# LeapLabTHU/LAUDNet

Hardware: AMD Instinct MI355X
Metric: images/sec, LAUD-ResNet101 @224 bs256 (dynamic-inference hot path) (higher is better)
Workload: dtype bf16x3 (fp32 tensors; each fp32 product = 3 bf16 MFMA products of hi/lo splits, fp32 accumulate)

## Files before the change

### include/ldn_hip.h

```cpp
#ifndef LDN_HIP_H
#define LDN_HIP_H

#include <stddef.h>
#include <stdint.h>

#ifdef __cplusplus
extern "C" {
#endif

#define LDN_OK 0
#define LDN_EINVAL (-1)
#define LDN_EHIP (-2)

const char* ldn_last_error(void);
int ldn_version(void);
int ldn_debug_violations(int* count, int* first_code, int reset);
int ldn_plan_timeouts(int* count, int reset);
const int* ldn_fault_flag(void);
int ldn_device_cus(int* cus);
#define LDN_MATH_DEFAULT (-1)
#define LDN_MATH_FP32 0
#define LDN_MATH_BF16X3 1
int ldn_default_math_mode(void);

int ldn_spatial_masker(const float* x, int B, int Hi, int Wi, int C, const float* w ,
                       const float* bias , int g, int S, float* mask, float* logits, float* work,
                       const int32_t* carry_prefix, const float* carry_mask, void* stream);
size_t ldn_spatial_masker_workspace_bytes(int B, int Hi, int Wi, int C, int S);

int ldn_mask_to_index(const float* patch_mask, int B, int Sy, int Sx, int Ho, int Wo, int stride, int32_t* idx3,
                      int32_t* pos3, int32_t* idx1, int32_t* pos1, int32_t* nbr, int32_t* cnt,
                      int32_t* img_prefix3, int32_t* img_prefix1, float* stats, int32_t* work, void* stream);
size_t ldn_mask_to_index_workspace_bytes(int B, int Ho, int Wo, int stride);
int ldn_plan_work_zeroed(int yes);
int ldn_coarsen_cell_means(const float* fine, int B, int S, int C, float* coarse, void* stream);

int ldn_layer_index(const float* image_mask, int B, int Ho, int Wo, int stride, int tile_gy, int tile_gx, int32_t* idx3,
                    int32_t* pos3, int32_t* idx1, int32_t* pos1, int32_t* nbr, int32_t* cnt, int32_t* img_prefix3,
                    int32_t* img_prefix1, float* stats, void* stream);
int ldn_layer_head(const float* pool, int B, int nparts, int C, const float* w , const float* bias , int g,
                   float* mask , float* logits , void* stream);
int ldn_mask_plan_fits(int S, int Sx, int Ho, int Wo, int stride);
int ldn_mask_plan(const float* patch_mask, const float* pool, int C, const float* w, const float* bias, float* mask_out,
                  float* logits, int B, int S, int Sx, int Ho, int Wo, int stride, int patch_major, int32_t* idx3,
                  int32_t* pos3, int32_t* idx1, int32_t* pos1, int32_t* nbr, int32_t* cnt, int32_t* img_prefix3,
                  int32_t* img_prefix1, float* stats, int32_t* work, void* stream);

int ldn_gather_rows(const float* src, int ld_src, const int32_t* rows, const int32_t* count, int cap, int C,
                    float* packed, int ld_packed, void* stream);
int ldn_scatter_add_relu(const float* packed, int ld_packed, const int32_t* rows, const int32_t* count, int cap,
                         int C, const float* identity, int ld_id, float* out, int ld_out, void* stream);

int ldn_conv_rows(const float* a, int lda, const int32_t* a_rows, int taps, const int32_t* m_count, int m_cap,
                  const float* w, int cin, int cout, const float* scale, const float* shift, int relu,
                  const int32_t* relu_if_neg, const int32_t* out_rows, const float* residual, int ldr,
                  float* out, int ldo, int math_mode, void* stream);

int ldn_conv_rows_split(const float* a, int lda, const int32_t* a_rows, int taps, const int32_t* m_count, int m_cap,
                        const void* w_split, int cin, int cout, const float* scale, const float* shift, int relu,
                        const int32_t* relu_if_neg, const int32_t* out_rows, const float* residual, int ldr, float* out,
                        int ldo, const float* post_sub, const float* chan_mask, int rows_per_image, int shift_classes,
                        const int32_t* pix_map, int Hi, int Wi, int Ho, int Wo, int stride, const float* ln_stats,
                        const float* ln_c1, void* stream);
int ldn_conv_rows_f32(const float* a, int lda, const int32_t* a_rows, int taps, const int32_t* m_count, int m_cap,
                        const float* w, int cin, int cout, const float* scale, const float* shift, int relu,
                        const int32_t* relu_if_neg, const int32_t* out_rows, const float* residual, int ldr, float* out,
                        int ldo, const float* post_sub, const float* chan_mask, int rows_per_image, int shift_classes,
                        const int32_t* pix_map, int Hi, int Wi, int Ho, int Wo, int stride, const float* ln_stats,
                        const float* ln_c1, void* stream);

int ldn_hint_rows(int rows);

int ldn_wgrad_rows_ok(int cin, int cout, int taps);
size_t ldn_wgrad_rows_workspace_bytes(int m_cap, int cin, int cout, int taps);
int ldn_wgrad_rows(const float* dy, int lddy, const float* a, int lda, int a_valid, const int32_t* a_rows, int taps,
                   const int32_t* m_count, int m_cap, int cin, int cout, float* dw, float* work, int math_mode, void* stream);

int ldn_rows_chanmask(float* u, int ldu, const int32_t* row_prefix, int B, const float* chan_mask, const int32_t* m_count, int m_cap,
                      int C, void* stream);

size_t ldn_rows_act_bwd_workspace_bytes(int m_cap, int C, int B);
int ldn_rows_act_bwd(const float* dh, int lddh, const float* u, int ldu, const float* post_sub, const float* scale, const float* shift,
                     const float* chan_mask, const int32_t* row_prefix, int B, const float* zy, int ldzy, const int32_t* m_count,
                     int m_cap, int C, float* du, int lddu, float* g_shift, float* g_scale_num, float* g_mask, float* work,
                     void* stream);

int ldn_conv_rows_pool(const float* a, int lda, const int32_t* a_rows, const int32_t* m_count, int m_cap, const void* w,
                       int cin, int cout, const float* scale, const float* shift, int relu, const int32_t* relu_if_neg,
                       const int32_t* out_rows, const float* residual, int ldr, float* out, int ldo, float* pool, int S,
                       int Sx, int Ho, int Wo, int math_mode, void* stream);

int ldn_conv_rows_ps(const float* a, int lda, int a_presplit, const int32_t* a_rows, const int32_t* m_count, int m_cap,
                     const void* w_split, int cin, int cout, const float* scale, const float* shift, int relu,
                     const int32_t* relu_if_neg, const int32_t* out_rows, const float* residual, int ldr, float* out, int ldo,
                     int out_presplit, float* pool, int S, int Sx, int Ho, int Wo, void* stream);
int ldn_conv3x3_rows_ps(const void* a_presplit, int lda, const int32_t* nbr, const int32_t* m_count, int m_cap, const void* w_split,
                        int cin, int cout, const float* scale, const float* shift, int relu, void* out, int ldo, int out_presplit,
                        int rows_hint, void* stream);
int ldn_row_stats(const float* x, int ld, int rows, int C, float eps, float* stats, void* stream);
int ldn_row_stats_list(const float* x, int ld, int rows, int C, float eps, const int32_t* list, const int32_t* count, float* stats,
                       void* stream);

int ldn_channel_masker_splits(int HW);
int ldn_channel_masker(const float* x, int B, int HW, int C, const float* w1, const float* b1, const float* w2,
                       const float* b2, int hidden, int G, int gran, const float* mask_in, float* mask,
                       float* logits, int32_t* ch_idx, int32_t* ch_cnt, float* work, const float* gap_partial,
                       int gap_splits, void* stream);
size_t ldn_channel_masker_workspace_bytes(int B, int HW, int C);

int ldn_forward_stats(const int32_t* cnt, int B, const float* denom, const float* st_in, int st_cols, const double* terms,
                      double static_flops, int n_blocks, float* st_out, float* perc, float* flops, void* stream);

int ldn_conv_image(const float* a, int lda, int B, int Hi, int Wi, int ksize, int stride, int Ho, int Wo,
                   const float* w, int cin, int cout, const int32_t* k_idx, const int32_t* k_cnt, int kgran,
                   const int32_t* n_idx, const int32_t* n_cnt, const float* scale, const float* shift,
                   int shift_classes, const float* post_sub, int relu, const float* residual, int ldr,
                   float* out, int ldo, float* colsum, int out_format, int math_mode, void* stream);

int ldn_bottleneck_head(const float* x, int ldx, int B, int HW, int cin, const void* w1_split, int width,
                        const int32_t* ch_idx, const int32_t* ch_cnt, const float* scale1, const float* shift1,
                        const float* post_sub1, void* h1_split, int ldh, void* stream);
int ldn_bottleneck_head_f32(const float* x, int ldx, int B, int HW, int cin, const float* w1, int width,
                            const int32_t* ch_idx, const int32_t* ch_cnt, const float* scale1, const float* shift1,
                            const float* post_sub1, float* h1, int ldh, void* stream);
int ldn_bottleneck_tail_f32(const void* h1, int ldh, int B, int H, int Wd, int stride, int width, const void* w2_pairs_f32,
                            const void* w3_pairs_f32, int cout, const int32_t* ch_idx, const int32_t* ch_cnt, const float* scale2,
                            const float* shift2_tab, const float* post_sub2, const float* shift3, const float* residual,
                            int ldr, float* out, int ldo, float* colsum, void* stream);
int ldn_bottleneck_tail_splits(int H, int Wd, int width, int stride);
int ldn_bottleneck_tail(const void* h1_split, int ldh, int B, int H, int Wd, int stride, int width, const void* w2_pairs,
                        const void* w3_pairs, int cout, const int32_t* ch_idx, const int32_t* ch_cnt, const float* scale2,
                        const float* shift2_tab, const float* post_sub2, const float* shift3, const float* residual,
                        int ldr, float* out, int ldo, float* colsum, void* stream);
size_t ldn_x_split_bytes(size_t pixels, int cin);
int ldn_bottleneck_head_split(const float* x, int ldx, int B, int HW, int cin, const void* w1_split, int width,
                              const int32_t* ch_idx, const int32_t* ch_cnt, const float* scale1, const float* shift1,
                              const float* post_sub1, void* h1_split, int ldh, void* x_split, void* stream);
int ldn_bottleneck_tail_proj_fits(int H, int Wd, int width, int cin);
int ldn_bottleneck_tail_proj(const void* h1_split, int ldh, int B, int H, int Wd, int width, const void* w2_pairs,
                             const void* w3_pairs, int cout, const int32_t* ch_idx, const int32_t* ch_cnt, const float* scale2,
                             const float* shift2_tab, const float* post_sub2, const float* shift3d, const void* x_split,
                             int cin, const void* wd_pairs, float* out, int ldo, float* colsum, void* stream);

int ldn_bottleneck_smallmap_fits(int H, int Wd, int cin, int width, int cout);
int ldn_bottleneck_smallmap(const float* x, int ldx, int B, int H, int Wd, int cin, int width, const void* w1_split,
                            const void* w2_pairs, const void* w3_pairs, int cout, const int32_t* ch_idx, const int32_t* ch_cnt,
                            const float* scale1, const float* shift1, const float* post_sub1, const float* scale2,
                            const float* shift2_tab, const float* post_sub2, const float* shift3, const float* residual, int ldr,
                            float* out, int ldo, float* colsum, void* stream);

typedef struct ldn_chain_block {
    const void* w1_split; const float* scale1; const float* shift1; const float* post_sub1;
    const void* w2_pairs; const void* w3_pairs; const float* scale2; const float* shift2_tab; const float* post_sub2;
    const float* shift3;
    const float* mw1; const float* mb1; const float* mw2; const float* mb2;
} ldn_chain_block;
int ldn_bottleneck_chain_fits(int H, int Wd, int C, int width, int hidden, int G);
int ldn_bottleneck_chain(const float* x_in, float* x_work, int ldx, int B, int H, int Wd, int C, int width,
                         const ldn_chain_block* blocks, int nblocks, int hidden, int G, int gran, const float* gap_in,
                         int gap_splits, float* colsum, float* masks, int32_t* ch_idx, int32_t* ch_cnt, void* h1_split,
                         int ldh, void* stream);
int ldn_bottleneck_chain_f32(const float* x_in, float* x_work, int ldx, int B, int H, int Wd, int C, int width,
                         const ldn_chain_block* blocks, int nblocks, int hidden, int G, int gran, const float* gap_in,
                         int gap_splits, float* colsum, float* masks, int32_t* ch_idx, int32_t* ch_cnt, float* h1,
                         int ldh, void* stream);

size_t ldn_stem_weight_bytes(int cout);
int ldn_stem_conv_pool(const float* x, int B, int H, int W, const void* w_frag, const float* shift, int cout, float* out,
                       int Hp, int Wp, void* stream);
int ldn_stem_gap_splits(int H, int W);
int ldn_stem_conv_pool_gap(const float* x, int B, int H, int W, const void* w_frag, const float* shift, int cout,
                           float* out, int Hp, int Wp, float* gap, void* stream);

size_t ldn_stem3_weight_bytes(int cout);
int ldn_stem3_conv(const float* x, int B, int H, int W, const void* w_frag, const float* shift, int cout, int relu, float* out,
                   int Ho, int Wo, void* stream);

int ldn_conv_packed(const float* a, int lda, int B, const int32_t* row_prefix, const int32_t* m_count, int m_cap,
                    const int32_t* a_map, int taps, const int32_t* out_map, const int32_t* pix_map, int Hi, int Wi,
                    int Ho, int Wo, int stride, const float* w, int cin, int cout, const int32_t* k_idx,
                    const int32_t* k_cnt, int kgran, const int32_t* n_idx, const int32_t* n_cnt, const float* scale,
                    const float* shift, int shift_classes, const float* post_sub, int relu,
                    const int32_t* relu_if_neg, const float* residual, int ldr, float* out, int ldo, int math_mode,
                    void* stream);

int ldn_grouped_conv3x3_rows(const float* a, int lda, const int32_t* nbr, const int32_t* m_count, int m_cap,
                             const float* w, int C, int group_width, const float* scale, const float* shift, int relu,
                             float* out, int ldo, void* stream);
size_t ldn_grouped16_weight_bytes(int C);
int ldn_grouped16_conv3x3_rows(const float* a, int lda, const int32_t* nbr, const int32_t* m_count, int m_cap,
                               const void* w_frag, int C, const float* scale, const float* shift, int relu, float* out,
                               int ldo, void* stream);

int ldn_grouped16_images_fit(int Hi, int Wi, int C);
int ldn_grouped16_conv3x3_images(const float* a, int lda, const int32_t* m_count, int images_cap, int Hi, int Wi, int Ho, int Wo,
                                 int stride, const void* w_frag, int C, const float* scale, const float* shift, int relu, float* out,
                                 int ldo, void* stream);
int ldn_grouped_conv3x3_image(const float* a, int lda, int B, int Hi, int Wi, int stride, int Ho, int Wo, const float* w,
                              int C, int group_width, const int32_t* ch_idx, const int32_t* ch_cnt, const float* scale,
                              const float* shift, int relu, float* out, int ldo, void* stream);
int ldn_se_packed(float* a, int lda, const int32_t* row_prefix, int B, int C, int S, const float* w1, const float* b1,
                  const float* w2, const float* b2, const int32_t* ch_idx, const int32_t* ch_cnt, int max_rows_per_image,
                  float* work, void* stream);
size_t ldn_se_packed_workspace_bytes(int B, int C, int max_rows_per_image);

int ldn_grouped16_images_bands(int Hi, int Wi, int Ho, int stride, int C);
int ldn_grouped16_conv3x3_images_gap(const float* a, int lda, const int32_t* m_count, int images_cap, int Hi, int Wi, int Ho, int Wo,
                                     int stride, const void* w_frag, int C, const float* scale, const float* shift, int relu, float* out,
                                     int ldo, float* gap_partial, void* stream);
int ldn_se_gate_slots(const float* gap_partial, int splits, const int32_t* m_count, int images_cap, int rows_per_image, int C, int S,
                      const float* w1, const float* b1, const float* w2, const float* b2, float* gate, void* stream);
int ldn_conv_rows_gated(const float* a, int lda, const int32_t* m_count, int m_cap, const void* w_split, int cin, int cout,
                        const float* scale, const float* shift, int relu, const int32_t* relu_if_neg, const int32_t* out_rows,
                        const float* residual, int ldr, float* out, int ldo, const float* gate, int gate_rows, void* stream);

int ldn_packed_mha(const float* qkv, int ld_qkv, const int32_t* tok_rows, const int32_t* img_prefix, int B, int heads,
                   int head_dim, int max_tokens, float scale, float* out, int ldo, void* stream);
int ldn_packed_mha_heads(const float* qkv, int ld_qkv, const int32_t* tok_rows, const int32_t* img_prefix, int B, int heads,
                         int head_dim, int max_tokens, float scale, const float* head_keep, float* out, int ldo, void* stream);

#ifdef __cplusplus
}
#endif
#endif
```

### laudnet_amd/_lib.py

```python
from __future__ import annotations

import ctypes as C
import os

import torch

_PKG = os.path.dirname(os.path.abspath(__file__))
LIB_PATH = os.environ.get("LDN_LIB_PATH", os.path.join(_PKG, "libldn_hip.so"))

_P = C.c_void_p
_I = C.c_int

SIGNATURES = {
    "ldn_last_error": ([], C.c_char_p),
    "ldn_version": ([], _I),
    "ldn_debug_violations": ([C.POINTER(_I), C.POINTER(_I), _I], _I),
    "ldn_plan_timeouts": ([C.POINTER(_I), _I], _I),
    "ldn_fault_flag": ([], C.POINTER(_I)),
    "ldn_device_cus": ([C.POINTER(_I)], _I),
    "ldn_default_math_mode": ([], _I),
    "ldn_spatial_masker": ([_P, _I, _I, _I, _I, _P, _P, _I, _I, _P, _P, _P, _P, _P, _P], _I),
    "ldn_spatial_masker_workspace_bytes": ([_I, _I, _I, _I, _I], C.c_size_t),
    "ldn_mask_to_index": ([_P, _I, _I, _I, _I, _I, _I, _P, _P, _P, _P, _P, _P, _P, _P, _P, _P, _P], _I),
    "ldn_mask_to_index_workspace_bytes": ([_I, _I, _I, _I], C.c_size_t),
    "ldn_mask_plan_fits": ([_I, _I, _I, _I, _I], _I),
    "ldn_hint_rows": ([_I], _I),
    "ldn_layer_index": ([_P, _I, _I, _I, _I, _I, _I, _P, _P, _P, _P, _P, _P, _P, _P, _P, _P], _I),
    "ldn_layer_head": ([_P, _I, _I, _I, _P, _P, _I, _P, _P, _P], _I),
    "ldn_mask_plan": ([_P, _P, _I, _P, _P, _P, _P, _I, _I, _I, _I, _I, _I, _I, _P, _P, _P, _P, _P, _P, _P, _P, _P, _P, _P], _I),
    "ldn_conv_rows_pool": ([_P, _I, _P, _P, _I, _P, _I, _I, _P, _P, _I, _P, _P, _P, _I, _P, _I, _P, _I, _I, _I, _I, _I, _P], _I),
    "ldn_conv_rows_ps": ([_P, _I, _I, _P, _P, _I, _P, _I, _I, _P, _P, _I, _P, _P, _P, _I, _P, _I, _I, _P, _I, _I, _I, _I, _P], _I),
    "ldn_conv3x3_rows_ps": ([_P, _I, _P, _P, _I, _P, _I, _I, _P, _P, _I, _P, _I, _I, _I, _P], _I),
    "ldn_gather_rows": ([_P, _I, _P, _P, _I, _I, _P, _I, _P], _I),
    "ldn_scatter_add_relu": ([_P, _I, _P, _P, _I, _I, _P, _I, _P, _I, _P], _I),
    "ldn_conv_rows": ([_P, _I, _P, _I, _P, _I, _P, _I, _I, _P, _P, _I, _P, _P, _P, _I, _P, _I, _I, _P], _I),
    "ldn_conv_rows_split": ([_P, _I, _P, _I, _P, _I, _P, _I, _I, _P, _P, _I, _P, _P, _P, _I, _P, _I, _P, _P, _I, _I, _P, _I, _I, _I,
                             _I, _I, _P, _P, _P], _I),
    "ldn_conv_rows_f32": ([_P, _I, _P, _I, _P, _I, _P, _I, _I, _P, _P, _I, _P, _P, _P, _I, _P, _I, _P, _P, _I, _I, _P, _I, _I, _I,
                             _I, _I, _P, _P, _P], _I),
    "ldn_wgrad_rows_ok": ([_I, _I, _I], _I),
    "ldn_wgrad_rows_workspace_bytes": ([_I, _I, _I, _I], C.c_size_t),
    "ldn_wgrad_rows": ([_P, _I, _P, _I, _I, _P, _I, _P, _I, _I, _I, _P, _P, _I, _P], _I),
    "ldn_rows_chanmask": ([_P, _I, _P, _I, _P, _P, _I, _I, _P], _I),
    "ldn_rows_act_bwd_workspace_bytes": ([_I, _I, _I], C.c_size_t),
    "ldn_rows_act_bwd": ([_P, _I, _P, _I, _P, _P, _P, _P, _P, _I, _P, _I, _P, _I, _I, _P, _I, _P, _P, _P, _P, _P], _I),
    "ldn_row_stats": ([_P, _I, _I, _I, C.c_float, _P, _P], _I),
    "ldn_row_stats_list": ([_P, _I, _I, _I, C.c_float, _P, _P, _P, _P], _I),
    "ldn_channel_masker_splits": ([_I], _I),
    "ldn_channel_masker": ([_P, _I, _I, _I, _P, _P, _P, _P, _I, _I, _I, _P, _P, _P, _P, _P, _P, _P, _I, _P], _I),
    "ldn_channel_masker_workspace_bytes": ([_I, _I, _I], C.c_size_t),
    "ldn_forward_stats": ([_P, _I, _P, _P, _I, _P, C.c_double, _I, _P, _P, _P, _P], _I),
    "ldn_conv_packed": ([_P, _I, _I, _P, _P, _I, _P, _I, _P, _P, _I, _I, _I, _I, _I, _P, _I, _I, _P, _P, _I, _P, _P, _P, _P,
                         _I, _P, _I, _P, _P, _I, _P, _I, _I, _P], _I),
    "ldn_grouped_conv3x3_rows": ([_P, _I, _P, _P, _I, _P, _I, _I, _P, _P, _I, _P, _I, _P], _I),
    "ldn_grouped16_weight_bytes": ([_I], C.c_size_t),
    "ldn_grouped16_conv3x3_rows": ([_P, _I, _P, _P, _I, _P, _I, _P, _P, _I, _P, _I, _P], _I),
    "ldn_grouped16_images_fit": ([_I, _I, _I], _I),
    "ldn_grouped16_conv3x3_images": ([_P, _I, _P, _I, _I, _I, _I, _I, _I, _P, _I, _P, _P, _I, _P, _I, _P], _I),
    "ldn_plan_work_zeroed": ([_I], _I),
    "ldn_coarsen_cell_means": ([_P, _I, _I, _I, _P, _P], _I),
    "ldn_grouped16_images_bands": ([_I, _I, _I, _I, _I], _I),
    "ldn_grouped16_conv3x3_images_gap": ([_P, _I, _P, _I, _I, _I, _I, _I, _I, _P, _I, _P, _P, _I, _P, _I, _P, _P], _I),
    "ldn_se_gate_slots": ([_P, _I, _P, _I, _I, _I, _I, _P, _P, _P, _P, _P, _P], _I),
    "ldn_conv_rows_gated": ([_P, _I, _P, _I, _P, _I, _I, _P, _P, _I, _P, _P, _P, _I, _P, _I, _P, _I, _P], _I),
    "ldn_grouped_conv3x3_image": ([_P, _I, _I, _I, _I, _I, _I, _I, _P, _I, _I, _P, _P, _P, _P, _I, _P, _I, _P], _I),
    "ldn_se_packed": ([_P, _I, _P, _I, _I, _I, _P, _P, _P, _P, _P, _P, _I, _P, _P], _I),
    "ldn_se_packed_workspace_bytes": ([_I, _I, _I], C.c_size_t),
    "ldn_conv_image": ([_P, _I, _I, _I, _I, _I, _I, _I, _I, _P, _I, _I, _P, _P, _I, _P, _P, _P, _P, _I, _P, _I,
                        _P, _I, _P, _I, _P, _I, _I, _P], _I),
    "ldn_bottleneck_head": ([_P, _I, _I, _I, _I, _P, _I, _P, _P, _P, _P, _P, _P, _I, _P], _I),
    "ldn_bottleneck_head_f32": ([_P, _I, _I, _I, _I, _P, _I, _P, _P, _P, _P, _P, _P, _I, _P], _I),
    "ldn_bottleneck_tail_splits": ([_I, _I, _I, _I], _I),
    "ldn_bottleneck_tail": ([_P, _I, _I, _I, _I, _I, _I, _P, _P, _I, _P, _P, _P, _P, _P, _P, _P, _I, _P, _I, _P, _P], _I),
    "ldn_bottleneck_tail_f32": ([_P, _I, _I, _I, _I, _I, _I, _P, _P, _I, _P, _P, _P, _P, _P, _P, _P, _I, _P, _I, _P, _P], _I),
    "ldn_x_split_bytes": ([C.c_size_t, _I], C.c_size_t),
    "ldn_bottleneck_head_split": ([_P, _I, _I, _I, _I, _P, _I, _P, _P, _P, _P, _P, _P, _I, _P, _P], _I),
    "ldn_bottleneck_tail_proj_fits": ([_I, _I, _I, _I], _I),
    "ldn_bottleneck_tail_proj": ([_P, _I, _I, _I, _I, _I, _P, _P, _I, _P, _P, _P, _P, _P, _P, _P, _I, _P, _P, _I, _P, _P], _I),
    "ldn_stem_weight_bytes": ([_I], C.c_size_t),
    "ldn_stem_conv_pool": ([_P, _I, _I, _I, _P, _P, _I, _P, _I, _I, _P], _I),
    "ldn_stem_gap_splits": ([_I, _I], _I),
    "ldn_stem_conv_pool_gap": ([_P, _I, _I, _I, _P, _P, _I, _P, _I, _I, _P, _P], _I),
    "ldn_stem3_weight_bytes": ([_I], C.c_size_t),
    "ldn_stem3_conv": ([_P, _I, _I, _I, _P, _P, _I, _I, _P, _I, _I, _P], _I),
    "ldn_packed_mha": ([_P, _I, _P, _P, _I, _I, _I, _I, C.c_float, _P, _I, _P], _I),
    "ldn_packed_mha_heads": ([_P, _I, _P, _P, _I, _I, _I, _I, C.c_float, _P, _P, _I, _P], _I),
    "ldn_bottleneck_chain_fits": ([_I, _I, _I, _I, _I, _I], _I),
    "ldn_bottleneck_smallmap_fits": ([_I, _I, _I, _I, _I], _I),
    "ldn_bottleneck_smallmap": ([_P, _I, _I, _I, _I, _I, _I, _P, _P, _P, _I, _P, _P, _P, _P, _P, _P, _P, _P, _P, _P, _I, _P, _I, _P, _P], _I),
    "ldn_bottleneck_chain": ([_P, _P, _I, _I, _I, _I, _I, _I, _P, _I, _I, _I, _I, _P, _I, _P, _P, _P, _P, _P, _I, _P], _I),
    "ldn_bottleneck_chain_f32": ([_P, _P, _I, _I, _I, _I, _I, _I, _P, _I, _I, _I, _I, _P, _I, _P, _P, _P, _P, _P, _I, _P], _I),
}

_lib = None


class LdnError(RuntimeError):
    pass


def load():
    global _lib
    if _lib is not None:
        return _lib
    if not os.path.exists(LIB_PATH):
        raise LdnError(f"{LIB_PATH} not found: build it with `python -m laudnet_amd.build` "
                       "(laudnet_amd has no CPU or PyTorch fallback for the hot path)")
    lib = C.CDLL(LIB_PATH)
    for name, (argtypes, restype) in SIGNATURES.items():
        fn = getattr(lib, name)
        fn.argtypes = argtypes
        fn.restype = restype
    _lib = lib
    return lib


def ptr(t):
    if t is None:
        return None
    return C.c_void_p(t.data_ptr())


def stream_ptr(t=None):
    return C.c_void_p(torch.cuda.current_stream(t.device if t is not None else None).cuda_stream)


_SYNC_CALLS = os.environ.get("LDN_SYNC_CALLS", "0") != "0"
_n_calls = 0


_fault = None


def _arm_fault_flag():
    global _fault
    if _fault is None:
        p = load().ldn_fault_flag()
        _fault = p if p else False


def check(status: int, what: str, fault_ok: bool = False):
    if status != 0:
        msg = load().ldn_last_error()
        raise LdnError(f"{what} failed ({status}): {msg.decode() if msg else '?'}")
    if _fault and not fault_ok and _fault[0] != 0:
        raise LdnError(f"{what}: a device-side bounded wait ran into its time bound since the last reset -- results computed since are "
                       "invalid (ops.plan_timeouts() counts the events, ops.plan_timeouts(reset=True) re-arms)")
    if _SYNC_CALLS:
        global _n_calls
        import sys
        import torch
        _n_calls += 1
        print(f"[ldn] {_n_calls} {what} ...", end="", file=sys.stderr, flush=True)
        if torch.cuda.is_current_stream_capturing():
            print(" (capturing)", file=sys.stderr, flush=True)
            return
        torch.cuda.synchronize()
        print(" ok", file=sys.stderr, flush=True)


def require_device(*tensors):
    cur = None
    for t in tensors:
        if t is None:
            continue
        if not t.is_cuda:
            raise LdnError("laudnet_amd ops need tensors on a HIP device (cuda:N); there is no CPU path")
        if cur is None:
            cur = torch.cuda.current_device()
            if _fault is None:
                _arm_fault_flag()
        if t.device.index != cur:
            raise LdnError(f"tensor on {t.device} but the current device is cuda:{cur}: wrap the call in "
                           f"torch.cuda.device({t.device.index}) (kernels are launched on the current device's stream)")
```

### laudnet_amd/csrc/ldn_tail.hip

```cpp
#include "ldn_common.h"
#include "ldn_mlp.h"
#include <type_traits>
#include <stdlib.h>

namespace ldn {

typedef __bf16 bf16x8 __attribute__((ext_vector_type(8)));
typedef unsigned u32x2 __attribute__((ext_vector_type(2)));
typedef unsigned u32x4 __attribute__((ext_vector_type(4)));

struct TailArgs {
    const unsigned char* h1; long h1_row_bytes;
    int B, Hi, Wi, Ho, Wo, W, cout;
    const unsigned char* w2p;
    const unsigned char* w3p;
    const int32_t* k_idx; const int32_t* k_cnt;
    const float* sc2; const float* sh2; const float* ps2;
    const float* sh3;
    const float* residual; int ldr; float* out; int ldo;
    float* colsum;
    int rows_per_blk, mblocks;
    int slice_bytes;
    const unsigned char* pxs; const unsigned char* pw;
};
constexpr int T_PROJ_CIN = 64;

__device__ __attribute__((aligned(16))) float g_tail_zero[4] = {0.f, 0.f, 0.f, 0.f};

#ifndef LDN_TAIL_PRIO
#define LDN_TAIL_PRIO 0
#endif
#ifdef LDN_TRACE
__device__ unsigned long long* g_tail_trace = nullptr;
__device__ unsigned long long* g_chain_trace = nullptr;
__device__ unsigned long long* g_head_trace = nullptr;
#define TT(x) x = __builtin_amdgcn_s_memtime();
#define TT_ADD(acc, a, b) acc += (b) - (a);
#else
#define TT(x)
#define TT_ADD(acc, a, b)
#endif

#ifndef LDN_TAIL_ABLATE
#define LDN_TAIL_ABLATE 0
#endif
#if LDN_TAIL_ABLATE & 4
template <typename A, typename B, typename C> __device__ __forceinline__ C t_mfma_bf16(A a, B b, C c) { asm volatile("" ::"v"(a), "v"(b)); return c; }
#else
#define t_mfma_bf16(a, b, c) __builtin_amdgcn_mfma_f32_32x32x16_bf16(a, b, c, 0, 0, 0)
#endif

__device__ __forceinline__ void dma16(const void* gsrc, unsigned lds_base) {
#if LDN_TAIL_ABLATE & 1
    return;
#endif
    unsigned keep;
    asm volatile("s_mov_b32 %0, m0\n\ts_mov_b32 m0, %2\n\ts_nop 0\n\tglobal_load_lds_dwordx4 %1, off\n\ts_mov_b32 m0, %0"
                 : "=&s"(keep) : "v"(gsrc), "s"(lds_base) : "memory");
}
__device__ __forceinline__ void dma4_touch(const void* gsrc, unsigned lds_base) {
    unsigned keep;
    asm volatile("s_mov_b32 %0, m0\n\ts_mov_b32 m0, %2\n\ts_nop 0\n\tglobal_load_lds_dword %1, off\n\ts_mov_b32 m0, %0"
                 : "=&s"(keep) : "v"(gsrc), "s"(lds_base) : "memory");
}
template <int N> __device__ __forceinline__ void wait_vm() {
    static_assert(N == 0 || N == 1 || N == 2 || N == 4, "add the immediate");
    if constexpr (N == 0) asm volatile("s_waitcnt vmcnt(0)" ::: "memory");
    else if constexpr (N == 1) asm volatile("s_waitcnt vmcnt(1)" ::: "memory");
    else if constexpr (N == 2) asm volatile("s_waitcnt vmcnt(2)" ::: "memory");
    else asm volatile("s_waitcnt vmcnt(4)" ::: "memory");
}
__device__ __forceinline__ void lds_barrier() {
    asm volatile("s_waitcnt lgkmcnt(0)" ::: "memory");
    __builtin_amdgcn_s_barrier();
    asm volatile("" ::: "memory");
}
__device__ __forceinline__ unsigned lds_off(const void* ptr) {
    return (unsigned)(size_t)(const __attribute__((address_space(3))) void*)ptr;
}

__device__ __forceinline__ void split2(float v, __bf16& hi, __bf16& lo) {
    hi = (__bf16)v;
    lo = (__bf16)(v - (float)hi);
}

#define LDN_K16(F32_, ACC_, AH_, AL_, BH_, BL_) \
    if constexpr (F32_) { \
        const f32x4 ka0_ = __builtin_bit_cast(f32x4, AH_), ka1_ = __builtin_bit_cast(f32x4, AL_); \
        const f32x4 kb0_ = __builtin_bit_cast(f32x4, BH_), kb1_ = __builtin_bit_cast(f32x4, BL_); \
        _Pragma("unroll") for (int ki_ = 0; ki_ < 4; ++ki_) ACC_ = __builtin_amdgcn_mfma_f32_32x32x2f32(ka0_[ki_], kb0_[ki_], ACC_, 0, 0, 0); \
        _Pragma("unroll") for (int ki_ = 0; ki_ < 4; ++ki_) ACC_ = __builtin_amdgcn_mfma_f32_32x32x2f32(ka1_[ki_], kb1_[ki_], ACC_, 0, 0, 0); \
    } else { \
        ACC_ = t_mfma_bf16(AL_, BH_, ACC_); \
        ACC_ = t_mfma_bf16(AH_, BL_, ACC_); \
        ACC_ = t_mfma_bf16(AH_, BH_, ACC_); \
    }

constexpr int T_KIDX_BYTES = 1280;
constexpr int T_W2_SLOTS = 3;

#define LDN_TAIL_CHUNK_MFMA(WS_, HS_, TR_) {                                                                  \
            const unsigned char* ws = (WS_); \
            const unsigned rbase = (unsigned)(TR_) * 128u, rx = ((unsigned)(TR_) >> 1) & 7u; \
            bf16x8 bh[2], bl[2]; \
    _Pragma("unroll") \
            for (int half = 0; half < 2; ++half) { \
                const unsigned sl = 2u * (2u * half + h); \
                bh[half] = *reinterpret_cast<const bf16x8*>((HS_) + rbase + ((sl ^ rx) << 4)); \
                bl[half] = *reinterpret_cast<const bf16x8*>((HS_) + rbase + (((sl + 1) ^ rx) << 4)); \
            } \
    _Pragma("unroll") \
            for (int j = 0; j < NS; ++j) { \
                if (j < nsub) { \
                    u32x2 e0[4], e1[4]; \
    _Pragma("unroll") \
                    for (int q = 0; q < 4; ++q) e0[q] = *reinterpret_cast<const u32x2*>(ws + a_lane + q * W2_ROW + j * 256); \
    _Pragma("unroll") \
                    for (int q = 0; q < 4; ++q) e1[q] = *reinterpret_cast<const u32x2*>(ws + a_lane + (8 + q) * W2_ROW + j * 256); \
                     \
                     \
                    { \
                        const u32x4 ahu = F32 ? u32x4{e0[0][0], e0[0][1], e0[1][0], e0[1][1]} : u32x4{e0[0][0], e0[1][0], e0[2][0], e0[3][0]}; \
                        const u32x4 alu = F32 ? u32x4{e0[2][0], e0[2][1], e0[3][0], e0[3][1]} : u32x4{e0[0][1], e0[1][1], e0[2][1], e0[3][1]}; \
                        const bf16x8 ah = __builtin_bit_cast(bf16x8, ahu), al = __builtin_bit_cast(bf16x8, alu); \
                        LDN_K16(F32, acc[j], ah, al, bh[0], bl[0]) \
                    } \
                    { \
                        const u32x4 ahu = F32 ? u32x4{e1[0][0], e1[0][1], e1[1][0], e1[1][1]} : u32x4{e1[0][0], e1[1][0], e1[2][0], e1[3][0]}; \
                        const u32x4 alu = F32 ? u32x4{e1[2][0], e1[2][1], e1[3][0], e1[3][1]} : u32x4{e1[0][1], e1[1][1], e1[2][1], e1[3][1]}; \
                        const bf16x8 ah = __builtin_bit_cast(bf16x8, ahu), al = __builtin_bit_cast(bf16x8, alu); \
                        LDN_K16(F32, acc[j], ah, al, bh[1], bl[1]) \
                    } \
                    __builtin_amdgcn_sched_group_barrier(0x100, 8, 0); \
                    __builtin_amdgcn_sched_group_barrier(0x008, 6, 0); \
                } \
            } \
}

template <int NS, int ST = 1, bool PROJ = false, bool F32 = false>
__device__ __forceinline__ void tail_body(const TailArgs& p, const int b, const int mb, unsigned char* const smem, const int tid) {
    static_assert(!PROJ || (NS == 2 && ST == 1), "the folded projection exists for the 64-wide stride-1 block (stage 1's first block)");
    static_assert(!(PROJ && F32), "the folded projection is a bf16x3 form");
    constexpr int W = NS * 32;
    constexpr int SLICE_BUFS = ST == 2 ? 2 : (NS == 2 ? 1 : 2);
    constexpr int W2_ROW = NS * 256;
    constexpr int W2_SLOT = 16 * W2_ROW;
    constexpr int CW = (NS == 8 || PROJ) ? 32 : 64;
    constexpr int NCS = CW / 32;
    constexpr int W3_ROW = CW * 8;
    constexpr int RPI = 1024 / W3_ROW;
    constexpr int PROWS = PROJ ? T_PROJ_CIN / 2 : 0;
    constexpr int W3_SLOT = (W / 2 + PROWS) * W3_ROW;
    constexpr int NP = W;
    int* const s_kidx = reinterpret_cast<int*>(smem);
    unsigned char* const s_h1 = smem + T_KIDX_BYTES;
    unsigned char* const s_w2 = s_h1 + SLICE_BUFS * p.slice_bytes;
    unsigned char* const s_w3 = smem + T_KIDX_BYTES;
    float* const s_tab = reinterpret_cast<float*>(s_w3 + 2 * W3_SLOT);
    unsigned char* const s_scr = reinterpret_cast<unsigned char*>(s_tab + 18 * NP);

    int lane = tid & 63;
    const int wave = __builtin_amdgcn_readfirstlane(tid >> 6);
    int l31 = lane & 31, h = lane >> 5;
#ifdef LDN_TRACE
    unsigned long long tr0, tr1 = 0, tr2 = 0, tr3 = 0, tr4 = 0, ta = 0, tb = 0, w2wait = 0, w3wait = 0, w3bar = 0, w3epi = 0, w3k = 0;
    TT(tr0)
#endif
    const int y0 = mb * p.rows_per_blk;
    const int rows = min(p.rows_per_blk, p.Ho - y0);
    const int npix = rows * p.Wo;
    const int yin0 = max(ST * y0 - 1, 0), yin1 = min(ST * (y0 + rows - 1) + 1, p.Hi - 1);
    const int NR = (yin1 - yin0 + 1) * p.Wi;
    const int NRp = round_up(NR, 8);
    const int ZR = ST == 2 ? p.slice_bytes / 128 - 1 : NRp;
    int plo[4] = {0, 0, 0, 0}, pw[4] = {1, 1, 1, 1}, pn[4] = {0, 0, 0, 0}, clo[4] = {0, 0, 0, 0};
    if constexpr (ST == 2) {
#pragma unroll
        for (int g = 0; g < 4; ++g) {
            const int py = g >> 1, px = g & 1;
            const int rlo = py ? max(y0 - 1, 0) : y0;
            const int rhi = min(y0 + rows - 1, (p.Hi - 1 - py) >> 1);
            const int chi = min(p.Wo - 1, (p.Wi - 1 - px) >> 1);
            plo[g] = rlo; clo[g] = 0;
            pw[g] = max(chi + 1, 1);
            pn[g] = (rhi >= rlo && chi >= 0 && p.Hi - 1 - py >= 0 && p.Wi - 1 - px >= 0) ? (rhi - rlo + 1) * (chi + 1) : 0;
        }
    }
    const long in_row0 = (long)b * p.Hi * p.Wi + (long)yin0 * p.Wi;
    const long out_row0 = (long)b * p.Ho * p.Wo + (long)y0 * p.Wo;

    const int Kb = min(p.k_cnt[b], W);
    const int nsub = ceil_div(Kb, 32);
    const int Kp = nsub * 32;
    if (tid < W + 32) s_kidx[tid] = tid < Kb ? p.k_idx[(size_t)b * W + tid] : -1;
    LDN_DCHECK(p.k_cnt[b] >= 0 && p.k_cnt[b] <= W && (p.k_cnt[b] & 1) == 0, 301);
    if (tid < Kb) {
        const int ch = p.k_idx[(size_t)b * W + tid];
        LDN_DCHECK(ch >= 0 && ch < W, 302);
        LDN_DCHECK((tid & 1) ? (ch == p.k_idx[(size_t)b * W + tid - 1] + 1) : ((ch & 1) == 0), 303);
        LDN_DCHECK(tid == 0 || ch > p.k_idx[(size_t)b * W + tid - 1], 304);
    }
    if (tid < 32 * SLICE_BUFS) reinterpret_cast<float*>(s_h1 + (tid >> 5) * p.slice_bytes + ZR * 128)[tid & 31] = 0.f;
    __syncthreads();

    const int pm = wave * 32 + l31;
    const bool pvalid = pm < npix;
    const int oy = y0 + pm / p.Wo, ox = pm % p.Wo;
    int trow[9];
#pragma unroll
    for (int t = 0; t < 9; ++t) {
        const int iy = ST * oy + t / 3 - 1, ix = ST * ox + t % 3 - 1;
        const bool ok = pvalid && iy >= 0 && iy < p.Hi && ix >= 0 && ix < p.Wi;
        if constexpr (ST == 2) {
            const int g = (iy & 1) * 2 + (ix & 1);
            trow[t] = ok ? ((iy >> 1) - plo[g]) * pw[g] + ((ix >> 1) - clo[g]) : ZR;
        } else {
            trow[t] = ok ? (iy - yin0) * p.Wi + ix : ZR;
        }
    }
    const int cls = (((ST * oy - 1 < 0) | ((ST * oy + 1 >= p.Hi) << 1)) * 4 + ((ST * ox - 1 < 0) | ((ST * ox + 1 >= p.Wi) << 1)));

    const unsigned lds_h1 = lds_off(s_h1), lds_w2 = lds_off(s_w2), lds_w3 = lds_off(s_w3);
    auto dma_h1 = [&](int slice, int q) {
        const int r = q * 8 + (lane >> 3);
        const int lslot = (lane & 7) ^ ((r >> 1) & 7);
        const unsigned char* src = r < NR ? p.h1 + (in_row0 + r) * p.h1_row_bytes + slice * 128 + lslot * 16
                                          : reinterpret_cast<const unsigned char*>(g_tail_zero);
        dma16(src, lds_h1 + (slice % SLICE_BUFS) * p.slice_bytes + q * 1024);
    };
    const int n_w2 = NS == 2 ? 1 : (NS == 4 ? 2 : (Kp > 128 ? 4 : 2));
    long npo[NS == 8 ? 2 : 1];
#pragma unroll
    for (int e = 0; e < (NS == 8 ? 2 : 1); ++e) {
        const int v = (NS == 2 ? (lane & 31) : lane) + 64 * e;
        const int ch = 2 * v < Kb ? s_kidx[2 * v] : -1;
        npo[e] = ch >= 0 ? (long)(ch >> 1) * 16 : -1;
    }
    auto dma_plane = [&](int slice, int g, int buf, int q) {
        const int r = q * 8 + (lane >> 3);
        const int lslot = (lane & 7) ^ ((r >> 1) & 7);
        const int pr = r / pw[g], pc = r - pr * pw[g];
        const long pix = (long)b * p.Hi * p.Wi + (long)(2 * (plo[g] + pr) + (g >> 1)) * p.Wi + 2 * (clo[g] + pc) + (g & 1);
        const unsigned char* src = r < pn[g] ? p.h1 + pix * p.h1_row_bytes + slice * 128 + lslot * 16
                                             : reinterpret_cast<const unsigned char*>(g_tail_zero);
        dma16(src, lds_h1 + buf * p.slice_bytes + q * 1024);
    };
    auto dma_w2e = [&](int c, int s, int t, int e) {
        const unsigned slot = lds_w2 + (c % T_W2_SLOTS) * W2_SLOT;
        const int u = 2 * wave + (NS == 2 ? (lane >> 5) : e);
        const int kch = s_kidx[32 * s + 2 * u];
        const long rowoff = ((long)t * (W / 2) + (kch >> 1)) * (W / 2) * 16;
        if (NS == 2) {
            if (e == 1) return;
            const unsigned char* src = (kch >= 0 && npo[0] >= 0) ? p.w2p + rowoff + npo[0] : reinterpret_cast<const unsigned char*>(g_tail_zero);
            dma16(src, slot + 2 * wave * W2_ROW);
        } else if (NS == 4) {
            const unsigned char* src = (kch >= 0 && npo[0] >= 0) ? p.w2p + rowoff + npo[0] : reinterpret_cast<const unsigned char*>(g_tail_zero);
            dma16(src, slot + u * W2_ROW);
        } else {
#pragma unroll
            for (int f = 0; f < 2; ++f) {
                if (f == 1 && Kp <= 128) break;
                const unsigned char* src = (kch >= 0 && npo[f] >= 0) ? p.w2p + rowoff + npo[f] : reinterpret_cast<const unsigned char*>(g_tail_zero);
                dma16(src, slot + u * W2_ROW + f * 1024);
            }
        }
    };
    auto dma_w2x = [&](int c, int s, int t) { dma_w2e(c, s, t, 0); dma_w2e(c, s, t, 1); };
    auto dma_w2_dummy = [&](int c, int e) {
        const int n = NS == 2 ? (e == 0 ? 1 : 0) : (NS == 4 ? 1 : (Kp > 128 ? 2 : 1));
        for (int i = 0; i < n; ++i) dma16(g_tail_zero, lds_w2 + (c % T_W2_SLOTS) * W2_SLOT + (2 * wave) * W2_ROW);
    };
    auto dma_w2 = [&](int c) { dma_w2x(c, c / 9, c % 9); };
    auto wait_chunk = [&]() {
        if (n_w2 == 1) wait_vm<1>();
        else if (n_w2 == 2) wait_vm<2>();
        else wait_vm<4>();
    };

    f32x16 acc[NS];
#pragma unroll
    for (int j = 0; j < NS; ++j)
#pragma unroll
        for (int r = 0; r < 16; ++r) acc[j][r] = 0.f;

    const int nchunks = nsub * 9;
    const int nq = NRp / 8;
    const bool active = wave * 32 < npix;
    const unsigned a_lane = (unsigned)(4 * h * W2_ROW + l31 * 8);
    if constexpr (ST == 2) {
        constexpr int ORD[4] = {3, 1, 2, 0};
        constexpr int NTP[4] = {4, 2, 2, 1};
        constexpr int TAPS[4][4] = {{0, 2, 6, 8}, {3, 5, 3, 3}, {1, 7, 1, 1}, {4, 4, 4, 4}};
        auto tap_of = [&](int c) {
            constexpr int SEQ[9] = {0, 2, 6, 8, 3, 5, 1, 7, 4};
            return SEQ[c % 9];
        };
        if (nchunks > 0) {
            for (int q = wave; q < (pn[3] + 7) / 8; q += 8) dma_plane(0, 3, 0, q);
            dma_w2x(0, 0, tap_of(0));
            dma_w2x(1, 0, tap_of(1));
        }
        TT(tr1)
        int c = 0;
        for (int s = 0; s < nsub; ++s) {
#pragma unroll
            for (int o = 0; o < 4; ++o) {
                const int u = 4 * s + o;
                const unsigned char* hs = s_h1 + (u & 1) * p.slice_bytes;
                const int gn = ORD[(o + 1) & 3], sn = o == 3 ? s + 1 : s;
                const int npn = sn < nsub ? (pn[gn] + 7) / 8 : 0;
#pragma unroll
                for (int i = 0; i < NTP[o]; ++i) {
                    TT(ta)
                    wait_chunk();
                    lds_barrier();
                    TT(tb)
                    TT_ADD(w2wait, ta, tb)
                    for (int q = i * 8 + wave; q < npn; q += 8 * NTP[o]) dma_plane(sn, gn, (u + 1) & 1, q);
                    if (c + 2 < nchunks) dma_w2x(c + 2, (c + 2) / 9, tap_of(c + 2));
                    else { for (int e = 0; e < n_w2; ++e) dma16(g_tail_zero, lds_w2 + ((c + 2) % T_W2_SLOTS) * W2_SLOT + (2 * wave) * W2_ROW); }
                    if (active) LDN_TAIL_CHUNK_MFMA(s_w2 + (c % T_W2_SLOTS) * W2_SLOT, hs, trow[TAPS[o][i]])
                    ++c;
                }
            }
        }
    } else {
    if (nchunks > 0) {
        for (int q = wave; q < nq; q += 8) dma_h1(0, q);
        dma_w2(0);
        dma_w2(1);
    }
    TT(tr1)
#ifdef LDN_TAIL_HALF_MAJOR
    bf16x8 bh[2], bl[2];
    auto load_b_half = [&](const unsigned char* hs_, int tr, int half) {
        const unsigned rbase = (unsigned)tr * 128u, rx = ((unsigned)tr >> 1) & 7u;
        const unsigned sl = 2u * (2u * half + h);
        bh[half] = *reinterpret_cast<const bf16x8*>(hs_ + rbase + ((sl ^ rx) << 4));
        bl[half] = *reinterpret_cast<const bf16x8*>(hs_ + rbase + (((sl + 1) ^ rx) << 4));
    };
    for (int s = 0; s < nsub; ++s) {
        const unsigned char* hs = s_h1 + (s % SLICE_BUFS) * p.slice_bytes;
#pragma unroll
        for (int t = 0; t < 9; ++t) {
            const int c = 9 * s + t;
            TT(ta)
            wait_chunk();
            lds_barrier();
            if (SLICE_BUFS == 1 && t == 0 && s > 0) {
                for (int q = wave; q < nq; q += 8) dma_h1(s, q);
                wait_vm<0>();
                lds_barrier();
            }
            TT(tb)
            TT_ADD(w2wait, ta, tb)
            auto issue = [&](int g) {
                if (g == 0) {
                    if (SLICE_BUFS == 2 && s + 1 < nsub) { const int q = t * 8 + wave; if (q < nq) dma_h1(s + 1, q); }
                } else if (c + 2 < nchunks) {
                    dma_w2e(c + 2, (c + 2) / 9, (c + 2) % 9, g - 1);
                } else {
                    dma_w2_dummy(t + 2, g - 1);
                }
            };
            if (!active) { issue(0); issue(1); issue(2); continue; }
            if (t == 0) { load_b_half(hs, trow[0], 0); load_b_half(hs, trow[0], 1); }
            const unsigned char* ws = s_w2 + (t % T_W2_SLOTS) * W2_SLOT;
#pragma unroll
            for (int half = 0; half < 2; ++half) {
#pragma unroll
                for (int j = 0; j < NS; ++j) {
                    if (j < nsub) {
                        u32x2 e[4];
#pragma unroll
                        for (int q = 0; q < 4; ++q) e[q] = *reinterpret_cast<const u32x2*>(ws + a_lane + (8 * half + q) * W2_ROW + j * 256);
                        const u32x4 ahu = F32 ? u32x4{e[0][0], e[0][1], e[1][0], e[1][1]} : u32x4{e[0][0], e[1][0], e[2][0], e[3][0]};
                        const u32x4 alu = F32 ? u32x4{e[2][0], e[2][1], e[3][0], e[3][1]} : u32x4{e[0][1], e[1][1], e[2][1], e[3][1]};
                        const bf16x8 ah = __builtin_bit_cast(bf16x8, ahu), al = __builtin_bit_cast(bf16x8, alu);
                        LDN_K16(F32, acc[j], ah, al, bh[half], bl[half])
                        __builtin_amdgcn_sched_group_barrier(0x100, 4, 0);
                        __builtin_amdgcn_sched_group_barrier(0x008, F32 ? 8 : 3, 0);
                    }
                    if (j == 0) {
                        if (half == 0) { issue(0); issue(1); } else issue(2);
                    }
                }
                if (t < 8) load_b_half(hs, trow[t + 1], half);
            }
        }
    }
#else
    for (int s = 0; s < nsub; ++s) {
        const unsigned char* hs = s_h1 + (s % SLICE_BUFS) * p.slice_bytes;
#pragma unroll
        for (int t = 0; t < 9; ++t) {
            const int c = 9 * s + t;
            TT(ta)
            wait_chunk();
            lds_barrier();
            if (SLICE_BUFS == 1 && t == 0 && s > 0) {
                for (int q = wave; q < nq; q += 8) dma_h1(s, q);
                wait_vm<0>();
                lds_barrier();
            }
            TT(tb)
            TT_ADD(w2wait, ta, tb)
#if LDN_TAIL_PRIO == 2
            __builtin_amdgcn_s_setprio(2);
#endif
            if (SLICE_BUFS == 2 && s + 1 < nsub) { const int q = t * 8 + wave; if (q < nq) dma_h1(s + 1, q); }
            if (c + 2 < nchunks) dma_w2(c + 2);
            else { for (int e = 0; e < n_w2; ++e) dma16(g_tail_zero, lds_w2 + ((t + 2) % T_W2_SLOTS) * W2_SLOT + (2 * wave) * W2_ROW); }
#if LDN_TAIL_PRIO == 2
            __builtin_amdgcn_s_setprio(0);
#endif
            if (!active) continue;
#if LDN_TAIL_PRIO == 1
            __builtin_amdgcn_s_setprio(1);
#endif
            LDN_TAIL_CHUNK_MFMA(s_w2 + (t % T_W2_SLOTS) * W2_SLOT, hs, trow[t])
#if LDN_TAIL_PRIO == 1
            __builtin_amdgcn_s_setprio(0);
#endif
        }
    }
#endif
    }
    wait_vm<0>();
    lds_barrier();
    TT(tr2)
    asm volatile("" : "+v"(lane));
    l31 = lane & 31;
    h = lane >> 5;

    const int nchunk3 = p.cout / CW;
    auto dma_w3 = [&](int cc) {
        const unsigned slot = lds_w3 + (cc & 1) * W3_SLOT;
        constexpr int LPR = 64 / RPI;
        for (int i = wave; i < Kp / (2 * RPI); i += 8) {
            const int u = RPI * i + lane / LPR;
            const int kch = s_kidx[2 * u];
            const unsigned char* src = kch >= 0 ? p.w3p + ((long)(kch >> 1) * p.cout + cc * CW + 2 * (lane % LPR)) * 8
                                                : reinterpret_cast<const unsigned char*>(g_tail_zero);
            dma16(src, slot + i * 1024);
        }
        if constexpr (PROJ) {
            for (int i = wave; i < PROWS / RPI; i += 8) {
                const int u = RPI * i + lane / LPR;
                const int r = u & 7;
                const int sp = (u & ~7) | ((r & 1) | ((r & 2) << 1) | ((r & 4) >> 1));
                dma16(p.pw + ((long)sp * p.cout + cc * CW + 2 * (lane % LPR)) * 8, slot + (Kp / (2 * RPI) + i) * 1024);
            }
        }
    };
    if (nchunk3 > 0) dma_w3(0);

    for (int i = tid; i < NP; i += 512) {
        const int ch = i < Kb ? s_kidx[i] : -1;
        const float a = p.sc2[max(ch, 0)], c = p.ps2[max(ch, 0)];
        s_tab[i] = ch >= 0 ? a : 0.f;
        s_tab[NP + i] = ch >= 0 ? c : 0.f;
    }
    {
        constexpr int TB = (16 * NP / 512) < 4 ? (16 * NP / 512) : 4;
        for (int i0 = tid; i0 < 16 * NP; i0 += 512 * TB) {
            float v[TB];
#pragma unroll
            for (int u = 0; u < TB; ++u) {
                const int i = i0 + 512 * u;
                const int k = i / NP, n = i - k * NP;
                const int ch = n < Kb ? s_kidx[n] : -1;
                const float x = p.sh2[k * W + max(ch, 0)];
                v[u] = ch >= 0 ? x : 0.f;
            }
#pragma unroll
            for (int u = 0; u < TB; ++u) s_tab[2 * NP + i0 + 512 * u] = v[u];
        }
    }
    lds_barrier();
    typedef __bf16 bf16x2 __attribute__((ext_vector_type(2)));
#pragma unroll
    for (int j = 0; j < NS; ++j) {
        float v[16];
#pragma unroll
        for (int q4 = 0; q4 < 4; ++q4) {
            const int n0 = 32 * j + 8 * q4 + 4 * h;
            const f32x4 sc = *reinterpret_cast<const f32x4*>(s_tab + n0);
            const f32x4 ps = *reinterpret_cast<const f32x4*>(s_tab + NP + n0);
            const f32x4 sh = *reinterpret_cast<const f32x4*>(s_tab + 2 * NP + cls * NP + n0);
#pragma unroll
            for (int e = 0; e < 4; ++e)
                v[4 * q4 + e] = fmaxf(acc[j][4 * q4 + e] * sc[e] + sh[e], 0.f) - ps[e];
        }
        if constexpr (F32) {
#pragma unroll
            for (int r = 0; r < 16; ++r) acc[j][r] = v[r];
        } else {
#pragma unroll
        for (int t = 0; t < 2; ++t)
#pragma unroll
            for (int d = 0; d < 4; ++d) {
                const float x0 = v[8 * t + 2 * d], x1 = v[8 * t + 2 * d + 1];
                const bf16x2 hi = {(__bf16)x0, (__bf16)x1};
                const bf16x2 lo = {(__bf16)(x0 - (float)hi[0]), (__bf16)(x1 - (float)hi[1])};
                acc[j][8 * t + d] = __builtin_bit_cast(float, hi);
                acc[j][8 * t + 4 + d] = __builtin_bit_cast(float, lo);
            }
        }
        asm volatile("" : "+v"(acc[j]) :: "memory");
        __builtin_amdgcn_sched_barrier(0);
    }
    auto frag_hi = [&](int j, int t) -> bf16x8 {
        const f32x4 x = {acc[j][8 * t], acc[j][8 * t + 1], acc[j][8 * t + 2], acc[j][8 * t + 3]};
        return __builtin_bit_cast(bf16x8, x);
    };
    auto frag_lo = [&](int j, int t) -> bf16x8 {
        const f32x4 x = {acc[j][8 * t + 4], acc[j][8 * t + 5], acc[j][8 * t + 6], acc[j][8 * t + 7]};
        return __builtin_bit_cast(bf16x8, x);
    };

    TT(tr3)
    const int trw = lane >> 3, tc = lane & 7;
    const unsigned a3_lane = (unsigned)(2 * h * W3_ROW + l31 * 8);
    float* const scr = reinterpret_cast<float*>(s_scr + wave * 4096);
    bf16x8 pjh[PROJ ? T_PROJ_CIN / 16 : 1], pjl[PROJ ? T_PROJ_CIN / 16 : 1];
    if constexpr (PROJ) {
        const long q = out_row0 + min(wave * 32 + l31, npix - 1);
        const unsigned char* xr = p.pxs + (q >> 5) * ((long)T_PROJ_CIN * 128) + (q & 31) * 16 + h * 1024;
#pragma unroll
        for (int s2 = 0; s2 < T_PROJ_CIN / 16; ++s2) {
            pjh[s2] = *reinterpret_cast<const bf16x8*>(xr + s2 * 2048);
            pjl[s2] = *reinterpret_cast<const bf16x8*>(xr + s2 * 2048 + 512);
        }
    }
    for (int cc = 0; cc < nchunk3; ++cc) {
        if (cc == 0) { wait_vm<0>(); lds_barrier(); }
        if (cc + 1 < nchunk3) dma_w3(cc + 1);
        const unsigned char* ws = s_w3 + (cc & 1) * W3_SLOT;
#pragma unroll
        for (int cs = 0; cs < NCS; ++cs) {
            const int c0 = cc * CW + cs * 32;
            f32x4 res[PROJ ? 1 : 4];
            if constexpr (!PROJ) {
#pragma unroll
            for (int it = 0; it < 4; ++it) {
                const int prow = wave * 32 + trw + 8 * it;
                const float* src = (p.residual && prow < npix) ? p.residual + (size_t)(out_row0 + prow) * p.ldr + c0 + tc * 4 : g_tail_zero;
                res[it] = __builtin_nontemporal_load(reinterpret_cast<const f32x4*>(src));
            }
            }
            f32x4 sh = *reinterpret_cast<const f32x4*>(p.sh3 + c0 + tc * 4);
            f32x16 acc3;
            TT(ta)
#pragma unroll
            for (int r = 0; r < 16; ++r) acc3[r] = 0.f;
#pragma unroll
            for (int j = 0; j < NS; ++j) {
                if (j < nsub && active) {
                    u32x2 e[2][4];
#pragma unroll
                    for (int t = 0; t < 2; ++t)
#pragma unroll
                        for (int q = 0; q < 4; ++q)
                            e[t][q] = *reinterpret_cast<const u32x2*>(ws + a3_lane + (16 * j + 8 * t + (q & 1) + 4 * (q >> 1)) * W3_ROW + cs * 256);
#pragma unroll
                    for (int t = 0; t < 2; ++t) {
                        const u32x4 ahu = F32 ? u32x4{e[t][0][0], e[t][0][1], e[t][1][0], e[t][1][1]} : u32x4{e[t][0][0], e[t][1][0], e[t][2][0], e[t][3][0]};
                        const u32x4 alu = F32 ? u32x4{e[t][2][0], e[t][2][1], e[t][3][0], e[t][3][1]} : u32x4{e[t][0][1], e[t][1][1], e[t][2][1], e[t][3][1]};
                        const bf16x8 ah = __builtin_bit_cast(bf16x8, ahu), al = __builtin_bit_cast(bf16x8, alu);
                        const bf16x8 hb = frag_hi(j, t), lb = frag_lo(j, t);
                        LDN_K16(F32, acc3, ah, al, hb, lb)
                    }
                    __builtin_amdgcn_sched_group_barrier(0x100, 8, 0);
                    __builtin_amdgcn_sched_group_barrier(0x008, 6, 0);
                }
            }
            if constexpr (PROJ) {
                if (active) {
#pragma unroll
                    for (int jj = 0; jj < T_PROJ_CIN / 32; ++jj) {
                        u32x2 e[2][4];
#pragma unroll
                        for (int t = 0; t < 2; ++t)
#pragma unroll
                            for (int q = 0; q < 4; ++q)
                                e[t][q] = *reinterpret_cast<const u32x2*>(ws + a3_lane + (Kp / 2 + 16 * jj + 8 * t + (q & 1) + 4 * (q >> 1)) * W3_ROW + cs * 256);
#pragma unroll
                        for (int t = 0; t < 2; ++t) {
                            const u32x4 ahu = {e[t][0][0], e[t][1][0], e[t][2][0], e[t][3][0]};
                            const u32x4 alu = {e[t][0][1], e[t][1][1], e[t][2][1], e[t][3][1]};
                            const bf16x8 ah = __builtin_bit_cast(bf16x8, ahu), al = __builtin_bit_cast(bf16x8, alu);
                            acc3 = t_mfma_bf16(al, pjh[2 * jj + t], acc3);
                            acc3 = t_mfma_bf16(ah, pjl[2 * jj + t], acc3);
                            acc3 = t_mfma_bf16(ah, pjh[2 * jj + t], acc3);
                        }
                        __builtin_amdgcn_sched_group_barrier(0x100, 8, 0);
                        __builtin_amdgcn_sched_group_barrier(0x008, 6, 0);
                    }
                }
            }
            TT(tb)
            TT_ADD(w3k, ta, tb)
            if (cs == NCS - 1) wait_vm<0>();
            if constexpr (PROJ) asm volatile("" : "+v"(sh));
            else asm volatile("" : "+v"(res[0]), "+v"(res[PROJ ? 0 : 1]), "+v"(res[PROJ ? 0 : 2]), "+v"(res[PROJ ? 0 : 3]), "+v"(sh));
            TT(ta)
            TT_ADD(w3wait, tb, ta)
#pragma unroll
            for (int q4 = 0; q4 < 4; ++q4) {
                const f32x4 v = {acc3[4 * q4], acc3[4 * q4 + 1], acc3[4 * q4 + 2], acc3[4 * q4 + 3]};
                *reinterpret_cast<f32x4*>(scr + l31 * 32 + (((2 * q4 + h) ^ (l31 & 7)) << 2)) = v;
            }
            asm volatile("s_waitcnt lgkmcnt(0)" ::: "memory");
            __builtin_amdgcn_wave_barrier();
            f32x4 csum = {0.f, 0.f, 0.f, 0.f};
#pragma unroll
            for (int it = 0; it < 4; ++it) {
                const int row = trw + 8 * it, prow = wave * 32 + row;
                f32x4 x = *reinterpret_cast<const f32x4*>(scr + row * 32 + ((tc ^ (row & 7)) << 2));
                if constexpr (PROJ) x = x + sh;
                else x = x + sh + res[PROJ ? 0 : it];
#pragma unroll
                for (int e = 0; e < 4; ++e) x[e] = fmaxf(x[e], 0.f);
                if (prow < npix) {
                    __builtin_nontemporal_store(x, reinterpret_cast<f32x4*>(p.out + (size_t)(out_row0 + prow) * p.ldo + c0 + tc * 4));
                    csum += x;
                }
            }
            if (p.colsum) {
#pragma unroll
                for (int e = 0; e < 4; ++e) csum[e] = sum_lane_bits_345(csum[e]);
                if (trw == 0)
                    *reinterpret_cast<f32x4*>(p.colsum + ((size_t)b * (p.mblocks * 8) + mb * 8 + wave) * p.cout + c0 + tc * 4) = csum;
            }
            asm volatile("s_waitcnt lgkmcnt(0)" ::: "memory");
            __builtin_amdgcn_wave_barrier();
            TT(tb)
            TT_ADD(w3epi, ta, tb)
        }
        TT(ta)
        lds_barrier();
        TT(tb)
        TT_ADD(w3bar, ta, tb)
    }
#ifdef LDN_TRACE
    TT(tr4)
    if (g_tail_trace && lane == 0) {
        unsigned long long* r = g_tail_trace + (((size_t)mb * p.B + b) * 8 + wave) * 12;
        r[0] = tr0; r[1] = tr1; r[2] = tr2; r[3] = tr3; r[4] = tr4; r[5] = w2wait; r[6] = w3k; r[7] = w3wait; r[8] = w3epi; r[9] = w3bar;
        r[10] = nsub; r[11] = 0;
    }
#endif
}

template <int NS, int ST, bool PROJ = false, bool F32 = false>
__global__ __launch_bounds__(512, ((NS == 2 && ST == 1) ? 4 : 2)) void k_tail(const TailArgs p) {
    extern __shared__ __attribute__((aligned(16))) unsigned char smem[];
    tail_body<NS, ST, PROJ, F32>(p, blockIdx.x % p.B, blockIdx.x / p.B, smem, threadIdx.x);
}

LDN_DEFINE_TU_VIOLATIONS(tu_violations_tail)

static int tail_region_pixels(int R, int Hi, int Wi, int st) {
    if (st == 2) return min(R + 1, (Hi + 1) / 2) * ((Wi - 1) / 2 + 1);
    return min(R + 2, Hi) * Wi;
}

static size_t tail_lds2(int R, int Hi, int Wi, int NS, int st) {
    const int nr = tail_region_pixels(R, Hi, Wi, st);
    const size_t slice = (size_t)round_up((round_up(nr, 8) + 1) * 128, 1024);
    return (size_t)T_KIDX_BYTES + (st == 2 ? 2 : (NS == 2 ? 1 : 2)) * slice + (size_t)T_W2_SLOTS * 16 * NS * 256;
}

static int tail_rows_per_block(int Hi, int Wi, int NS, int st, int* mblocks) {
    const int Ho = (Hi - 1) / st + 1, Wo = (Wi - 1) / st + 1;
    int R = 256 / Wo;
    if (R < 1) return 0;
    if (R > Ho) R = Ho;
    auto fits = [&](int r) {
        return tail_lds2(r, Hi, Wi, NS, st) <= 160 * 1024 && (st == 2 || NS == 2 || round_up(tail_region_pixels(r, Hi, Wi, st), 8) / 8 <= 72);
    };
    while (R > 1 && !fits(R)) --R;
    if (!fits(R)) return 0;
    const int mbk = ceil_div(Ho, R);
    *mblocks = mbk;
    int best = ceil_div(Ho, mbk), best_waves = 1 << 30;
    for (int r = ceil_div(Ho, mbk); r <= R; ++r) {
        if (r * (mbk - 1) >= Ho) break;
        int waves = 0;
        for (int i = 0; i < mbk; ++i) waves += ceil_div(min(r, Ho - r * i) * Wo, 32);
        if (waves < best_waves) { best_waves = waves; best = r; }
    }
    return best;
}

template <int NS, int ST, bool PROJ = false, bool F32 = false>
static int launch_tail(TailArgs& a, hipStream_t st) {
    constexpr int W = NS * 32;
    const int R = a.rows_per_blk;
    const int nr = tail_region_pixels(R, a.Hi, a.Wi, ST);
    a.slice_bytes = round_up((round_up(nr, 8) + 1) * 128, 1024);
    const size_t lds2 = tail_lds2(R, a.Hi, a.Wi, NS, ST);
    const size_t lds3 = (size_t)T_KIDX_BYTES + 2 * (size_t)(W / 2 + (PROJ ? T_PROJ_CIN / 2 : 0)) * ((NS == 8 || PROJ) ? 32 : 64) * 8 + (size_t)18 * W * 4 + 8 * 4096;
    const size_t lds = lds2 > lds3 ? lds2 : lds3;
    LDN_REQUIRE(lds <= 160 * 1024, "ldn_bottleneck_tail: %zu B of LDS exceed 160 KiB (map %dx%d, width %d)", lds, a.Ho, a.Wo, W);
    LDN_REQUIRE(ST == 2 || NS == 2 || round_up(nr, 8) / 8 <= 72, "ldn_bottleneck_tail: input region of %d pixels too large for the slice pipeline", nr);
    LDN_REQUIRE(allow_dynamic_lds(reinterpret_cast<const void*>(&k_tail<NS, ST, PROJ, F32>), lds), "k_tail: cannot reserve %zu B of LDS", lds);
    hipLaunchKernelGGL((k_tail<NS, ST, PROJ, F32>), dim3((unsigned)a.B * a.mblocks), dim3(512), lds, st, a);
    LDN_CHECK_LAUNCH("k_tail");
    return LDN_OK;
}

}

using namespace ldn;

#ifdef LDN_TRACE
extern "C" int ldn_debug_set_chain_trace(void* buf) {
    unsigned long long* q = static_cast<unsigned long long*>(buf);
    return hipMemcpyToSymbol(HIP_SYMBOL(g_chain_trace), &q, sizeof(q)) == hipSuccess ? 0 : -2;
}
extern "C" int ldn_debug_set_ld_trace(void* buf);
extern "C" int ldn_debug_set_head_trace(void* buf) {
    unsigned long long* q = static_cast<unsigned long long*>(buf);
    return hipMemcpyToSymbol(HIP_SYMBOL(g_head_trace), &q, sizeof(q)) == hipSuccess ? 0 : -2;
}
extern "C" int ldn_debug_set_tail_trace(void* buf) {
    unsigned long long* q = static_cast<unsigned long long*>(buf);
    return hipMemcpyToSymbol(HIP_SYMBOL(g_tail_trace), &q, sizeof(q)) == hipSuccess ? 0 : -2;
}
#endif

extern "C" int ldn_bottleneck_tail_splits(int H, int Wd, int width, int stride) {
    int mbk = 0;
    if (H < 1 || Wd < 1 || (stride != 1 && stride != 2) || (Wd - 1) / stride + 1 > 256 || (width != 64 && width != 128 && width != 256)) return 0;
    if (tail_rows_per_block(H, Wd, width / 32, stride, &mbk) == 0) return 0;
    return mbk * 8;
}

static int bottleneck_tail_impl(const void* h1_split, int ldh, int B, int H, int Wd, int stride, int width, const void* w2_pairs,
                                const void* w3_pairs, int cout, const int32_t* ch_idx, const int32_t* ch_cnt,
                                const float* scale2, const float* shift2_tab, const float* post_sub2,
                                const float* shift3, const float* residual, int ldr, float* out, int ldo,
                                float* colsum, const void* x_split, const void* wd_pairs, bool f32, void* stream);

extern "C" int ldn_bottleneck_tail(const void* h1_split, int ldh, int B, int H, int Wd, int stride, int width, const void* w2_pairs,
                                   const void* w3_pairs, int cout, const int32_t* ch_idx, const int32_t* ch_cnt,
                                   const float* scale2, const float* shift2_tab, const float* post_sub2,
                                   const float* shift3, const float* residual, int ldr, float* out, int ldo,
                                   float* colsum, void* stream) {
    return bottleneck_tail_impl(h1_split, ldh, B, H, Wd, stride, width, w2_pairs, w3_pairs, cout, ch_idx, ch_cnt, scale2, shift2_tab,
                                post_sub2, shift3, residual, ldr, out, ldo, colsum, nullptr, nullptr, false, stream);
}

extern "C" int ldn_bottleneck_tail_f32(const void* h1, int ldh, int B, int H, int Wd, int stride, int width, const void* w2_pairs_f32,
                                       const void* w3_pairs_f32, int cout, const int32_t* ch_idx, const int32_t* ch_cnt,
                                       const float* scale2, const float* shift2_tab, const float* post_sub2,
                                       const float* shift3, const float* residual, int ldr, float* out, int ldo,
                                       float* colsum, void* stream) {
    return bottleneck_tail_impl(h1, ldh, B, H, Wd, stride, width, w2_pairs_f32, w3_pairs_f32, cout, ch_idx, ch_cnt, scale2, shift2_tab,
                                post_sub2, shift3, residual, ldr, out, ldo, colsum, nullptr, nullptr, true, stream);
}

extern "C" int ldn_bottleneck_tail_proj_fits(int H, int Wd, int width, int cin) {
    int mbk = 0;
    if (H < 1 || Wd < 1 || Wd > 256 || width != 64 || cin != ldn::T_PROJ_CIN) return 0;
    return ldn::tail_rows_per_block(H, Wd, 2, 1, &mbk) > 0 ? 1 : 0;
}

extern "C" int ldn_bottleneck_tail_proj(const void* h1_split, int ldh, int B, int H, int Wd, int width, const void* w2_pairs,
                                        const void* w3_pairs, int cout, const int32_t* ch_idx, const int32_t* ch_cnt,
                                        const float* scale2, const float* shift2_tab, const float* post_sub2, const float* shift3d,
                                        const void* x_split, int cin, const void* wd_pairs, float* out, int ldo,
                                        float* colsum, void* stream) {
    LDN_REQUIRE(x_split && wd_pairs, "ldn_bottleneck_tail_proj: null pointer");
    LDN_REQUIRE(width == 64 && cin == ldn::T_PROJ_CIN, "ldn_bottleneck_tail_proj: the folded projection exists for width 64, cin 64 (got %d, %d; ldn_bottleneck_tail_proj_fits == 0)", width, cin);
    LDN_REQUIRE((uintptr_t)x_split % 16 == 0 && (uintptr_t)wd_pairs % 16 == 0, "ldn_bottleneck_tail_proj: x_split / wd_pairs must be 16-byte aligned");
    return bottleneck_tail_impl(h1_split, ldh, B, H, Wd, 1, width, w2_pairs, w3_pairs, cout, ch_idx, ch_cnt, scale2, shift2_tab,
                                post_sub2, shift3d, nullptr, 0, out, ldo, colsum, x_split, wd_pairs, false, stream);
}

static int bottleneck_tail_impl(const void* h1_split, int ldh, int B, int H, int Wd, int stride, int width, const void* w2_pairs,
                                const void* w3_pairs, int cout, const int32_t* ch_idx, const int32_t* ch_cnt,
                                const float* scale2, const float* shift2_tab, const float* post_sub2,
                                const float* shift3, const float* residual, int ldr, float* out, int ldo,
                                float* colsum, const void* x_split, const void* wd_pairs, bool f32, void* stream) {
    LDN_REQUIRE(h1_split && w2_pairs && w3_pairs && ch_idx && ch_cnt && scale2 && shift2_tab && post_sub2 && shift3 && out,
                "ldn_bottleneck_tail: null pointer");
    LDN_REQUIRE(width == 64 || width == 128 || width == 256, "ldn_bottleneck_tail: width must be 64, 128 or 256 (got %d)", width);
    LDN_REQUIRE(stride == 1 || stride == 2, "ldn_bottleneck_tail: stride must be 1 or 2 (got %d)", stride);
    LDN_REQUIRE(B > 0 && H > 0 && Wd > 0 && (Wd - 1) / stride + 1 <= 256, "ldn_bottleneck_tail: bad geometry (output map width must be <= 256)");
    LDN_REQUIRE(cout > 0 && cout % 64 == 0, "ldn_bottleneck_tail: cout must be a multiple of 64 (got %d)", cout);
    LDN_REQUIRE(ldh >= width && ldh % 8 == 0, "ldn_bottleneck_tail: ldh must be a multiple of 8 and >= width");
    LDN_REQUIRE(ldo >= cout && ldo % 4 == 0 && (!residual || (ldr >= cout && ldr % 4 == 0)), "ldn_bottleneck_tail: bad ldo / ldr");
    LDN_REQUIRE((uintptr_t)h1_split % 16 == 0 && (uintptr_t)w2_pairs % 16 == 0 && (uintptr_t)w3_pairs % 16 == 0 &&
                (uintptr_t)out % 16 == 0 && (uintptr_t)residual % 16 == 0 && (uintptr_t)shift3 % 16 == 0 && (uintptr_t)colsum % 16 == 0,
                "ldn_bottleneck_tail: pointers must be 16-byte aligned");
    LDN_REQUIRE((long)9 * (width / 2) * (width / 2) * 16 < (1L << 31), "ldn_bottleneck_tail: weights too large");
    TailArgs a{};
    a.h1 = static_cast<const unsigned char*>(h1_split);
    a.h1_row_bytes = (long)ldh * 4;
    a.B = B; a.Hi = H; a.Wi = Wd; a.Ho = (H - 1) / stride + 1; a.Wo = (Wd - 1) / stride + 1; a.W = width; a.cout = cout;
    a.w2p = static_cast<const unsigned char*>(w2_pairs);
    a.w3p = static_cast<const unsigned char*>(w3_pairs);
    a.k_idx = ch_idx; a.k_cnt = ch_cnt;
    a.sc2 = scale2; a.sh2 = shift2_tab; a.ps2 = post_sub2; a.sh3 = shift3;
    a.residual = residual; a.ldr = ldr; a.out = out; a.ldo = ldo; a.colsum = colsum;
    a.pxs = static_cast<const unsigned char*>(x_split); a.pw = static_cast<const unsigned char*>(wd_pairs);
    a.rows_per_blk = tail_rows_per_block(H, Wd, width / 32, stride, &a.mblocks);
    LDN_REQUIRE(a.rows_per_blk > 0, "ldn_bottleneck_tail: a %dx%d map of width %d (stride %d) does not fit the workgroup (ldn_bottleneck_tail_splits == 0)", H, Wd, width, stride);
    hipStream_t st = static_cast<hipStream_t>(stream);
    if (f32) {
        LDN_REQUIRE(!x_split, "ldn_bottleneck_tail: the folded projection is a bf16x3 form");
        if (stride == 2) {
            if (width == 64) return launch_tail<2, 2, false, true>(a, st);
            if (width == 128) return launch_tail<4, 2, false, true>(a, st);
            return launch_tail<8, 2, false, true>(a, st);
        }
        if (width == 64) return launch_tail<2, 1, false, true>(a, st);
        if (width == 128) return launch_tail<4, 1, false, true>(a, st);
        return launch_tail<8, 1, false, true>(a, st);
    }
    if (stride == 2) {
        if (width == 64) return launch_tail<2, 2>(a, st);
        if (width == 128) return launch_tail<4, 2>(a, st);
        return launch_tail<8, 2>(a, st);
    }
    if (x_split) return launch_tail<2, 1, true>(a, st);
    if (width == 64) return launch_tail<2, 1>(a, st);
    if (width == 128) return launch_tail<4, 1>(a, st);
    return launch_tail<8, 1>(a, st);
}

namespace ldn {

struct HeadArgs {
    const float* x; int ldx;
    int B, HW, cin, W;
    const unsigned char* w1s;
    const int32_t* n_idx; const int32_t* n_cnt;
    const float* sc1; const float* sh1; const float* ps1;
    unsigned char* h1; long h1_row_bytes;
    int pix_per_blk, mblocks;
    unsigned char* xs;
};

template <int N> __device__ __forceinline__ void wait_vm_n() {
    asm volatile("s_waitcnt vmcnt(%0)" ::"n"(N) : "memory");
}
__device__ __forceinline__ void wait_vm_rt(int n) {
    switch (n) {
        case 0: wait_vm_n<0>(); break;   case 1: wait_vm_n<1>(); break;   case 2: wait_vm_n<2>(); break;
        case 3: wait_vm_n<3>(); break;   case 4: wait_vm_n<4>(); break;   case 5: wait_vm_n<5>(); break;
        case 6: wait_vm_n<6>(); break;   case 7: wait_vm_n<7>(); break;   case 8: wait_vm_n<8>(); break;
        case 9: wait_vm_n<9>(); break;   case 10: wait_vm_n<10>(); break; case 11: wait_vm_n<11>(); break;
        case 12: wait_vm_n<12>(); break; case 13: wait_vm_n<13>(); break; case 14: wait_vm_n<14>(); break;
        case 15: wait_vm_n<15>(); break; default: wait_vm_n<16>(); break;
    }
}

template <int NF> __device__ __forceinline__ void dma16_pieces(const unsigned (&vo)[4], const void* sbase, unsigned lds_base) {
#if LDN_TAIL_ABLATE & 1
    return;
#endif
    unsigned keep;
    if constexpr (NF == 1)
        asm volatile("s_mov_b32 %0, m0\n\ts_mov_b32 m0, %3\n\ts_nop 0\n\tglobal_load_lds_dwordx4 %1, %2\n\ts_mov_b32 m0, %0"
                     : "=&s"(keep) : "v"(vo[0]), "s"(sbase), "s"(lds_base) : "memory");
    else if constexpr (NF == 2)
        asm volatile("s_mov_b32 %0, m0\n\ts_mov_b32 m0, %4\n\ts_nop 0\n\tglobal_load_lds_dwordx4 %1, %3\n\tglobal_load_lds_dwordx4 %2, %3 offset:1024\n\ts_mov_b32 m0, %0"
                     : "=&s"(keep) : "v"(vo[0]), "v"(vo[1]), "s"(sbase), "s"(lds_base) : "memory");
    else if constexpr (NF == 3)
        asm volatile("s_mov_b32 %0, m0\n\ts_mov_b32 m0, %5\n\ts_nop 0\n\tglobal_load_lds_dwordx4 %1, %4\n\tglobal_load_lds_dwordx4 %2, %4 offset:1024\n\t"
                     "global_load_lds_dwordx4 %3, %4 offset:2048\n\ts_mov_b32 m0, %0"
                     : "=&s"(keep) : "v"(vo[0]), "v"(vo[1]), "v"(vo[2]), "s"(sbase), "s"(lds_base) : "memory");
    else
        asm volatile("s_mov_b32 %0, m0\n\ts_mov_b32 m0, %6\n\ts_nop 0\n\tglobal_load_lds_dwordx4 %1, %5\n\tglobal_load_lds_dwordx4 %2, %5 offset:1024\n\t"
                     "global_load_lds_dwordx4 %3, %5 offset:2048\n\tglobal_load_lds_dwordx4 %4, %5 offset:3072\n\ts_mov_b32 m0, %0"
                     : "=&s"(keep) : "v"(vo[0]), "v"(vo[1]), "v"(vo[2]), "v"(vo[3]), "s"(sbase), "s"(lds_base) : "memory");
}
__device__ __forceinline__ const void* uniform_cptr(const void* v) {
    const unsigned long long u = reinterpret_cast<unsigned long long>(v);
    const unsigned lo = __builtin_amdgcn_readfirstlane((unsigned)u), hi = __builtin_amdgcn_readfirstlane((unsigned)(u >> 32));
    return reinterpret_cast<const void*>(((unsigned long long)hi << 32) | lo);
}

constexpr int H_XROWS = 256;

template <int NS, bool F32 = false, bool PRE_ROWS = false>
__device__ __forceinline__ void head_body(const HeadArgs& p, const int b, const int mb, unsigned char* const smem, const int lds_total, const int tid) {
    constexpr int W = NS * 32;
    int* const s_nidx = reinterpret_cast<int*>(smem);
    float* const s_tab = reinterpret_cast<float*>(smem + T_KIDX_BYTES);
    unsigned char* const s_ring = smem + T_KIDX_BYTES + 3 * W * 4;

    const int lane = tid & 63;
    const int wave = __builtin_amdgcn_readfirstlane(tid >> 6);
    const int l31 = lane & 31, h = lane >> 5;
    const int m0 = mb * p.pix_per_blk;
    const int npix = min(p.pix_per_blk, p.HW - m0);
    const long row0 = (long)b * p.HW + m0;

    const int Nb = min(p.n_cnt[b], W);
    const int nsub = __builtin_amdgcn_readfirstlane(ceil_div(Nb, 32));
    const int wrows = round_up(max(Nb, 1), 64);
    if (tid < W + 32) s_nidx[tid] = tid < Nb ? p.n_idx[(size_t)b * W + tid] : -1;
    __syncthreads();
    for (int i = tid; i < 3 * W; i += 512) {
        const int k = i / W, n = i - k * W;
        const int ch = s_nidx[n];
        const float* src = k == 0 ? p.sc1 : (k == 1 ? p.sh1 : p.ps1);
        s_tab[i] = ch >= 0 ? src[ch] : 0.f;
    }
    const int xrows = round_up(npix, 32);
    const int slot_bytes = (xrows + wrows) * 128;
#ifdef LDN_HEAD_L2PF
    constexpr int PF = 1;
#else
    constexpr int PF = 0;
#endif
    const int avail = lds_total - (T_KIDX_BYTES + 3 * W * 4) - 256;
    const int D = min(4, avail / slot_bytes);
    const int nchunks = p.cin / 32;
    const unsigned lds_ring = lds_off(s_ring);
    const int nw = wrows / 64;
    const bool active = wave * 32 < npix;
    const int per_chunk = (active ? 4 + PF : 0) + nw;

    unsigned xo[4], wo[4];
    {
        const int r8 = lane >> 3;
#pragma unroll
        for (int i = 0; i < 4; ++i) {
            const int r = wave * 32 + i * 8 + r8;
            const int ls = (lane & 7) ^ ((r >> 1) & 7);
            xo[i] = (unsigned)((min(r, npix - 1) * p.ldx + ls * 4) * 4 + (3 - i) * 1024);
            const int rw = i * 64 + wave * 8 + r8;
            const int lw = (lane & 7) ^ (r8 >> 1);
            const int ch = s_nidx[min(rw, max(Nb, 1) - 1)];
            wo[i] = (unsigned)(max(ch, 0) * p.cin * 4 + lw * 16 + (3 - i) * 1024);
        }
    }
    const unsigned char* const xbase = reinterpret_cast<const unsigned char*>(p.x + row0 * p.ldx) - 3072;
    const unsigned char* const wbase = p.w1s - 3072;
    auto dma_chunk = [&](int c) {
        const unsigned slot = lds_ring + (c % D) * slot_bytes;
        const int cc = min(c, nchunks - 1);
        if (active) dma16_pieces<4>(xo, uniform_cptr(xbase + (long)cc * 128), __builtin_amdgcn_readfirstlane(slot + wave * 32 * 128));
        if (PF && active) {
            const int pc = min(c + 2 + (lane >> 5), nchunks - 1);
            dma4_touch(reinterpret_cast<const unsigned char*>(p.x + (row0 + min(wave * 32 + l31, npix - 1)) * p.ldx) + (long)pc * 128,
                       __builtin_amdgcn_readfirstlane((unsigned)(lds_ring + (unsigned)avail)));
        }
        const void* wb = uniform_cptr(wbase + (long)cc * 128);
        const unsigned wl = __builtin_amdgcn_readfirstlane(slot + (xrows + wave * nw * 8) * 128);
        if (nw == 1) dma16_pieces<1>(wo, wb, wl);
        else if (nw == 2) dma16_pieces<2>(wo, wb, wl);
        else if (nw == 3) dma16_pieces<3>(wo, wb, wl);
        else dma16_pieces<4>(wo, wb, wl);
    };
    auto dma_dummy = [&](int c) { dma_chunk(c); };

    f32x16 acc[NS];
#pragma unroll
    for (int j = 0; j < NS; ++j)
#pragma unroll
        for (int r = 0; r < 16; ++r) acc[j][r] = 0.f;

    for (int c = 0; c < D - 1; ++c) { if (c < nchunks) dma_chunk(c); else dma_dummy(c); }
    const unsigned xrow = (unsigned)(wave * 32 + l31), xsw = (xrow >> 1) & 7u;
    const unsigned wsw = ((unsigned)l31 >> 1) & 3u;
    const unsigned wrow_e = (unsigned)((((l31 >> 3)) * nw * 8 + (l31 & 7)) * 128);
    const unsigned wrow_o = (unsigned)((((4 + (l31 >> 3))) * nw * 8 + (l31 & 7)) * 128);
#ifdef LDN_TRACE
    unsigned long long h0, h1, h2, h3, h4, h5, hw = 0, hb = 0, hi_ = 0, hs = 0, hm = 0, hstart;
    TT(hstart)
#endif
    bf16x8 bh[2], bl[2];
    auto load_b = [&](int c) {
        const unsigned char* xs = s_ring + (c % D) * slot_bytes;
#pragma unroll
        for (int half = 0; half < 2; ++half) {
            const unsigned sl = 4u * half + 2u * h;
            const f32x4 x0 = *reinterpret_cast<const f32x4*>(xs + xrow * 128 + ((sl ^ xsw) << 4));
            const f32x4 x1 = *reinterpret_cast<const f32x4*>(xs + xrow * 128 + (((sl + 1) ^ xsw) << 4));
            if constexpr (F32) {
                bh[half] = __builtin_bit_cast(bf16x8, x0);
                bl[half] = __builtin_bit_cast(bf16x8, x1);
            } else {
#pragma unroll
                for (int e = 0; e < 8; ++e) {
                    const float v = e < 4 ? x0[e] : x1[e - 4];
                    const __bf16 hb = (__bf16)v;
                    bh[half][e] = hb;
                    bl[half][e] = (__bf16)(v - (float)hb);
                }
            }
        }
        if (!F32 && p.xs && (int)xrow < npix) {
            const long q = row0 + xrow;
            unsigned char* xo_ = p.xs + (q >> 5) * ((long)p.cin * 128) + (q & 31) * 16 + h * 1024;
#pragma unroll
            for (int half = 0; half < 2; ++half) {
                *reinterpret_cast<bf16x8*>(xo_ + (2 * c + half) * 2048) = bh[half];
                *reinterpret_cast<bf16x8*>(xo_ + (2 * c + half) * 2048 + 512) = bl[half];
            }
        }
    };
    constexpr bool PRE = PRE_ROWS;
    const int own_landed = per_chunk * (D - 1) - 4;
    if (PRE && active && nchunks > 0) {
        wait_vm_rt(own_landed);
        load_b(0);
    }
    for (int c = 0; c < nchunks; ++c) {
        TT(h0)
        wait_vm_rt(per_chunk * (D - 2));
        TT(h1)
        lds_barrier();
        TT(h2)
        if (c + D - 1 < nchunks) dma_chunk(c + D - 1); else dma_dummy(c + D - 1);
        TT(h3)
        TT_ADD(hw, h0, h1) TT_ADD(hb, h1, h2) TT_ADD(hi_, h2, h3)
        if (!active) continue;
        const unsigned char* ws = s_ring + (c % D) * slot_bytes + xrows * 128;
        if (!PRE) load_b(c);
#ifdef LDN_TRACE
        asm volatile("" : "+v"(bh[0]), "+v"(bl[0]), "+v"(bh[1]), "+v"(bl[1]));
        TT(h4)
        TT_ADD(hs, h3, h4)
#endif
        bf16x8 a0h, a0l, a1h, a1l;
        const unsigned sl0 = 2u * h, sl1 = 4u + 2u * h;
        auto frag0 = [&](int j) {
            const unsigned char* wr = ws + ((j & 1) ? wrow_o : wrow_e) + (j >> 1) * 1024;
            a0h = *reinterpret_cast<const bf16x8*>(wr + ((sl0 ^ wsw) << 4));
            a0l = *reinterpret_cast<const bf16x8*>(wr + (((sl0 + 1) ^ wsw) << 4));
        };
        auto frag1 = [&](int j) {
            const unsigned char* wr = ws + ((j & 1) ? wrow_o : wrow_e) + (j >> 1) * 1024;
            a1h = *reinterpret_cast<const bf16x8*>(wr + ((sl1 ^ wsw) << 4));
            a1l = *reinterpret_cast<const bf16x8*>(wr + (((sl1 + 1) ^ wsw) << 4));
        };
#define LDN_HEAD_STEP(J)                                                                                  \
        frag1(J);                                                                                         \
        __builtin_amdgcn_sched_barrier(0);                                                                \
        LDN_K16(F32, acc[J], a0h, a0l, bh[0], bl[0])                                                      \
        __builtin_amdgcn_sched_barrier(0);                                                                \
        if (J > 0) frag0(J > 0 ? J - 1 : 0);                                                              \
        __builtin_amdgcn_sched_barrier(0);                                                                \
        LDN_K16(F32, acc[J], a1h, a1l, bh[1], bl[1])                                                      \
        __builtin_amdgcn_sched_barrier(0);
        if (nsub > 0) {
            frag0(nsub - 1);
            switch (nsub) {
                default:
                    if constexpr (NS >= 8) { LDN_HEAD_STEP(7) }
                    [[fallthrough]];
                case 7:
                    if constexpr (NS >= 8) { LDN_HEAD_STEP(6) }
                    [[fallthrough]];
                case 6:
                    if constexpr (NS >= 8) { LDN_HEAD_STEP(5) }
                    [[fallthrough]];
                case 5:
                    if constexpr (NS >= 8) { LDN_HEAD_STEP(4) }
                    [[fallthrough]];
                case 4:
                    if constexpr (NS >= 4) { LDN_HEAD_STEP(3) }
                    [[fallthrough]];
                case 3:
                    if constexpr (NS >= 4) { LDN_HEAD_STEP(2) }
                    [[fallthrough]];
                case 2:
                    LDN_HEAD_STEP(1)
                    [[fallthrough]];
                case 1:
                    LDN_HEAD_STEP(0)
            }
        }
#undef LDN_HEAD_STEP
        if (PRE && c + 1 < nchunks) {
            wait_vm_rt(own_landed);
            load_b(c + 1);
        }
#ifdef LDN_TRACE
        asm volatile("" : "+v"(acc[0]));
        TT(h5)
        TT_ADD(hm, h4, h5)
#endif
    }
#ifdef LDN_TRACE
    if (g_head_trace && lane == 0) {
        unsigned long long hend;
        TT(hend)
        unsigned long long* r = g_head_trace + (((size_t)mb * p.B + b) * 8 + wave) * 8;
        r[0] = hw; r[1] = hb; r[2] = hi_; r[3] = hs; r[4] = hm; r[5] = hend - hstart; r[6] = nchunks; r[7] = nsub;
    }
#endif
    wait_vm_n<0>();

    const int pm = wave * 32 + l31;
    if (!active) return;
    unsigned char* orow = p.h1 + (row0 + min(pm, npix - 1)) * p.h1_row_bytes;
#pragma unroll
    for (int j = 0; j < NS; ++j) {
        if (j >= nsub) continue;
#pragma unroll
        for (int q4 = 0; q4 < 4; ++q4) {
            const int n0 = 32 * j + 8 * q4 + 4 * h;
            const f32x4 sc = *reinterpret_cast<const f32x4*>(s_tab + n0);
            const f32x4 sh = *reinterpret_cast<const f32x4*>(s_tab + W + n0);
            const f32x4 ps = *reinterpret_cast<const f32x4*>(s_tab + 2 * W + n0);
            if constexpr (F32) {
// ... 548 lines not shown
```

### laudnet_amd/ops.py

```python
from __future__ import annotations

import os
import threading
import weakref
from dataclasses import dataclass

import torch

from . import _lib as L


def _f32c(t, what):
    if t is None:
        return None
    if t.dtype != torch.float32 or not t.is_contiguous():
        raise L.LdnError(f"{what}: expected a contiguous float32 tensor, got {t.dtype} strides {t.stride()}")
    return t


def _f32rows(t, what):
    if t is None:
        return None
    if t.dtype != torch.float32 or t.dim() != 2 or t.stride(1) != 1 or t.data_ptr() % 16 != 0:
        raise L.LdnError(f"{what}: expected a 16-byte aligned float32 matrix with contiguous rows, got {t.dtype} strides {t.stride()}")
# ... 518 lines not shown
                                 L.ptr(_i32c(m_count, "m_count")), m_cap, L.ptr(split_rows_weight(w)), cin, cout,
                                 L.ptr(_f32c(scale, "scale")), L.ptr(_f32c(shift, "shift")), relu, L.ptr(_i32c(relu_if_neg, "relu_if_neg")),
                                 L.ptr(_i32c(out_rows, "out_rows")), L.ptr(_f32rows(residual2d, "residual")),
                                 residual2d.stride(0) if residual2d is not None else 0, L.ptr(_f32rows(out2d, "out")), out2d.stride(0),
                                 1 if out_presplit else 0, L.ptr(_f32c(pool, "pool")), S, Sx, ho, wo, L.stream_ptr(out2d)), "ldn_conv_rows_ps")
    return out2d


def conv3x3_rows_ps(a2d, nbr, w, scale, shift, out2d, *, m_count=None, m_cap=None, relu=1, out_presplit=False, rows_hint=None):
    L.require_device(a2d, nbr, w, out2d)
    lib = L.load()
    cout, t, cin = w.shape
    if t != 9:
        raise L.LdnError("conv3x3_rows_ps: 3x3 weights [cout, 9, cin] expected")
    if m_cap is None:
        m_cap = nbr.numel() // 9
    hint = int(rows_hint) if (rows_hint is not None and USE_ROWS_HINT) else -1
    L.check(lib.ldn_conv3x3_rows_ps(L.ptr(_f32rows(a2d, "a")), a2d.stride(0), L.ptr(_i32c(nbr, "nbr")), L.ptr(_i32c(m_count, "m_count")), m_cap,
                                    L.ptr(split_rows_weight(w)), cin, cout, L.ptr(_f32c(scale, "scale")), L.ptr(_f32c(shift, "shift")), relu,
                                    L.ptr(_f32rows(out2d, "out")), out2d.stride(0), 1 if out_presplit else 0, hint, L.stream_ptr(out2d)),
            "ldn_conv3x3_rows_ps")
    return out2d


def presplit_rows(x2d):
    rows, C = x2d.shape
    hi = x2d.to(torch.bfloat16)
    lo = (x2d - hi.float()).to(torch.bfloat16)
    packed = torch.stack((hi.view(rows, C // 8, 8), lo.view(rows, C // 8, 8)), dim=2).contiguous()
    return packed.view(torch.float32).reshape(rows, C)


def unsplit_rows(ps2d):
    rows, C = ps2d.shape
    b = ps2d.contiguous().view(torch.bfloat16).reshape(rows, C // 8, 2, 8).float()
    return (b[:, :, 0] + b[:, :, 1]).reshape(rows, C)


def channel_masker(x_nhwc, w1, b1, w2, b2, groups, gran, mask_in=None, want_logits=False, gap_partial=None, hw=None):
    lib = L.load()
    src = x_nhwc if x_nhwc is not None else (mask_in if mask_in is not None else gap_partial)
    dev = src.device
    L.require_device(x_nhwc, mask_in, gap_partial)
    if gap_partial is not None:
        x_nhwc = None
    gap_splits = 0
    if mask_in is not None:
        B = mask_in.shape[0]
        HW = C = hidden = 0
        work = None
    elif gap_partial is not None:
        B, gap_splits, C = gap_partial.shape
        HW = hw
        hidden = 0 if w2 is None else w1.shape[0]
        work = None
        _f32c(gap_partial, "gap_partial")
    else:
        B, H, W, C = x_nhwc.shape
        HW = H * W
        hidden = 0 if w2 is None else w1.shape[0]
        work = _work(lib.ldn_channel_masker_workspace_bytes(B, HW, C), dev)
    width = groups * gran
    mask = torch.empty(B, groups, device=dev, dtype=torch.float32)
    idx = torch.empty(B, width, device=dev, dtype=torch.int32)
    cnt = torch.empty(B, device=dev, dtype=torch.int32)
    logits = torch.empty(B, 2 * groups, device=dev, dtype=torch.float32) if (want_logits and mask_in is None) else None
    L.check(lib.ldn_channel_masker(L.ptr(x_nhwc), B, HW, C, L.ptr(w1), L.ptr(b1), L.ptr(w2), L.ptr(b2), hidden, groups,
                                   gran, L.ptr(_f32c(mask_in, "mask_in") if mask_in is not None else None), L.ptr(mask),
                                   L.ptr(logits), L.ptr(idx), L.ptr(cnt), L.ptr(work), L.ptr(gap_partial), gap_splits,
                                   L.stream_ptr()), "ldn_channel_masker")
    return mask, idx, cnt, logits


def conv_image(a_nhwc, w, scale, shift, out_nhwc, *, ksize=1, stride=1, k_idx=None, k_cnt=None, kgran=1, n_idx=None,
               n_cnt=None, post_sub=None, relu=1, residual=None, colsum=None, math=None, out_split=False):
    L.require_device(a_nhwc, w, out_nhwc)
    lib = L.load()
    B, Hi, Wi, lda = a_nhwc.shape
    _, Ho, Wo, ldo = out_nhwc.shape
    if k_idx is None:
        cout, t, cin = w.shape
    else:
        t, cin, cout = w.shape
    if t != ksize * ksize:
        raise L.LdnError("conv_image: weight taps do not match ksize")
    classes = 1 if shift.dim() == 1 else shift.shape[0]
    L.check(lib.ldn_conv_image(L.ptr(_f32c(a_nhwc, "a")), lda, B, Hi, Wi, ksize, stride, Ho, Wo, L.ptr(_f32c(w, "w")),
                               cin, cout, L.ptr(_i32c(k_idx, "k_idx")), L.ptr(_i32c(k_cnt, "k_cnt")), kgran,
                               L.ptr(_i32c(n_idx, "n_idx")), L.ptr(_i32c(n_cnt, "n_cnt")),
                               L.ptr(_f32c(scale, "scale")), L.ptr(_f32c(shift, "shift")), classes, L.ptr(post_sub),
                               relu, L.ptr(residual), residual.shape[-1] if residual is not None else 0,
                               L.ptr(_f32c(out_nhwc, "out")), ldo, L.ptr(colsum), 1 if out_split else 0, _mm(math),
                               L.stream_ptr(out_nhwc)),
            "ldn_conv_image")
    return out_nhwc


def conv_packed(a2d, w, scale, shift, out2d, *, B=1, row_prefix=None, m_count=None, m_cap=None, a_map=None, taps=1,
                out_map=None, pix_map=None, geom=None, k_idx=None, k_cnt=None, kgran=1, n_idx=None, n_cnt=None,
                post_sub=None, relu=1, relu_if_neg=None, residual2d=None, math=None):
    L.require_device(a2d, w, out2d)
    lib = L.load()
    if k_idx is None:
        cout, t, cin = w.shape
    else:
        t, cin, cout = w.shape
    if t != taps:
        raise L.LdnError(f"conv_packed: weight has {t} taps, expected {taps}")
    classes = 1 if shift.dim() == 1 else shift.shape[0]
    hi, wi, ho, wo, stride = geom if geom is not None else (0, 0, 0, 0, 1)
    L.check(lib.ldn_conv_packed(L.ptr(_f32c(a2d, "a")), a2d.stride(0), B, L.ptr(_i32c(row_prefix, "row_prefix")),
                                L.ptr(_i32c(m_count, "m_count")), m_cap, L.ptr(_i32c(a_map, "a_map")), taps,
                                L.ptr(_i32c(out_map, "out_map")), L.ptr(_i32c(pix_map, "pix_map")), hi, wi, ho, wo, stride,
                                L.ptr(_f32c(w, "w")), cin, cout, L.ptr(_i32c(k_idx, "k_idx")), L.ptr(_i32c(k_cnt, "k_cnt")),
                                kgran, L.ptr(_i32c(n_idx, "n_idx")), L.ptr(_i32c(n_cnt, "n_cnt")),
                                L.ptr(_f32c(scale, "scale")), L.ptr(_f32c(shift, "shift")), classes, L.ptr(post_sub), relu,
                                L.ptr(_i32c(relu_if_neg, "relu_if_neg")), L.ptr(residual2d),
                                residual2d.stride(0) if residual2d is not None else 0, L.ptr(_f32rows(out2d, "out")),
                                out2d.stride(0), _mm(math), L.stream_ptr(out2d)), "ldn_conv_packed")
    return out2d


def grouped_conv3x3_rows(a2d, nbr, w, group_width, scale, shift, out2d, *, m_count=None, m_cap=None, relu=1):
    L.require_device(a2d, nbr, w, out2d)
    lib = L.load()
    C = w.shape[0]
    m_cap = out2d.shape[0] if m_cap is None else m_cap
    L.check(lib.ldn_grouped_conv3x3_rows(L.ptr(_f32c(a2d, "a")), a2d.stride(0), L.ptr(_i32c(nbr, "nbr")),
                                         L.ptr(_i32c(m_count, "m_count")), m_cap, L.ptr(_f32c(w, "w")), C, group_width,
                                         L.ptr(_f32c(scale, "scale")), L.ptr(_f32c(shift, "shift")), relu,
                                         L.ptr(_f32c(out2d, "out")), out2d.stride(0), L.stream_ptr()),
            "ldn_grouped_conv3x3_rows")
    return out2d


def pack_grouped16_weights(w):
    C = w.shape[0]
    if tuple(w.shape[1:]) != (9, 16) or C % 16:
        raise L.LdnError("pack_grouped16_weights: expected [C % 16 == 0, 9, 16]")
    k = torch.zeros(C, 10, 16, device=w.device, dtype=torch.float32)
    k[:, :9] = w.detach().float()
    k = k.reshape(C // 16, 16, 5, 2, 2, 8)
    k = k.permute(0, 2, 3, 4, 1, 5).reshape(C // 16, 5, 64, 8)
    hi, lo = _hi_lo(k)
    return torch.stack((hi, lo), dim=-2).contiguous()


def grouped16_conv3x3_rows(a2d, nbr, w_frag, scale, shift, out2d, *, m_count=None, m_cap=None, relu=1):
    L.require_device(a2d, nbr, w_frag, out2d)
    lib = L.load()
    C = w_frag.shape[0] * 16
    if w_frag.dtype != torch.bfloat16 or not w_frag.is_contiguous() or w_frag.numel() * 2 != lib.ldn_grouped16_weight_bytes(C):
        raise L.LdnError("grouped16_conv3x3_rows: w_frag must be the contiguous bf16 tensor of pack_grouped16_weights")
    m_cap = out2d.shape[0] if m_cap is None else m_cap
    L.check(lib.ldn_grouped16_conv3x3_rows(L.ptr(_f32c(a2d, "a")), a2d.stride(0), L.ptr(_i32c(nbr, "nbr")),
                                           L.ptr(_i32c(m_count, "m_count")), m_cap, L.ptr(w_frag), C, L.ptr(_f32c(scale, "scale")),
                                           L.ptr(_f32c(shift, "shift")), relu, L.ptr(_f32c(out2d, "out")), out2d.stride(0),
                                           L.stream_ptr()), "ldn_grouped16_conv3x3_rows")
    return out2d


def grouped16_images_fit(Hi, Wi, C):
    return int(L.load().ldn_grouped16_images_fit(int(Hi), int(Wi), int(C)))


def grouped16_conv3x3_images(a2d, w_frag, scale, shift, out2d, *, m_count, images, relu=1):
    L.require_device(a2d, w_frag, out2d, m_count)
    lib = L.load()
    C = w_frag.shape[0] * 16
    if w_frag.dtype != torch.bfloat16 or not w_frag.is_contiguous() or w_frag.numel() * 2 != lib.ldn_grouped16_weight_bytes(C):
        raise L.LdnError("grouped16_conv3x3_images: w_frag must be the contiguous bf16 tensor of pack_grouped16_weights")
    B, Hi, Wi, Ho, Wo, stride = (int(v) for v in images)
    if a2d.shape[0] < B * Hi * Wi or out2d.shape[0] < B * Ho * Wo:
        raise L.LdnError("grouped16_conv3x3_images: a / out must hold B whole images")
    L.check(lib.ldn_grouped16_conv3x3_images(L.ptr(_f32c(a2d, "a")), a2d.stride(0), L.ptr(_i32c(m_count, "m_count")), B, Hi, Wi, Ho,
                                             Wo, stride, L.ptr(w_frag), C, L.ptr(_f32c(scale, "scale")),
                                             L.ptr(_f32c(shift, "shift")), relu, L.ptr(_f32c(out2d, "out")), out2d.stride(0),
                                             L.stream_ptr()), "ldn_grouped16_conv3x3_images")
    return out2d


def grouped16_images_bands(Hi, Wi, Ho, stride, C):
    return int(L.load().ldn_grouped16_images_bands(int(Hi), int(Wi), int(Ho), int(stride), int(C)))


def grouped16_conv3x3_images_gap(a2d, w_frag, scale, shift, out2d, *, m_count, images, relu=1):
    L.require_device(a2d, w_frag, out2d, m_count)
    lib = L.load()
    C = w_frag.shape[0] * 16
    if w_frag.dtype != torch.bfloat16 or not w_frag.is_contiguous() or w_frag.numel() * 2 != lib.ldn_grouped16_weight_bytes(C):
        raise L.LdnError("grouped16_conv3x3_images_gap: w_frag must be the contiguous bf16 tensor of pack_grouped16_weights")
    B, Hi, Wi, Ho, Wo, stride = (int(v) for v in images)
    if a2d.shape[0] < B * Hi * Wi or out2d.shape[0] < B * Ho * Wo:
        raise L.LdnError("grouped16_conv3x3_images_gap: a / out must hold B whole images")
    bands = grouped16_images_bands(Hi, Wi, Ho, stride, C)
    if bands <= 0:
        raise L.LdnError("grouped16_conv3x3_images_gap: the map does not fit the LDS (grouped16_images_fit)")
    gap = torch.empty(B, bands, C, device=a2d.device, dtype=torch.float32)
    L.check(lib.ldn_grouped16_conv3x3_images_gap(L.ptr(_f32c(a2d, "a")), a2d.stride(0), L.ptr(_i32c(m_count, "m_count")), B, Hi, Wi, Ho,
                                                 Wo, stride, L.ptr(w_frag), C, L.ptr(_f32c(scale, "scale")),
                                                 L.ptr(_f32c(shift, "shift")), relu, L.ptr(_f32c(out2d, "out")), out2d.stride(0),
                                                 L.ptr(gap), L.stream_ptr()), "ldn_grouped16_conv3x3_images_gap")
    return gap


def se_gate_slots(gap, m_count, rows_per_image, w1, b1, w2, b2):
    L.require_device(gap, m_count, w1)
    lib = L.load()
    B, bands, C = gap.shape
    S = w1.shape[0]
    gate = torch.empty(B, C, device=gap.device, dtype=torch.float32)
    L.check(lib.ldn_se_gate_slots(L.ptr(_f32c(gap, "gap")), bands, L.ptr(_i32c(m_count, "m_count")), B, int(rows_per_image), C, S,
                                  L.ptr(_f32c(w1, "w1")), L.ptr(_f32c(b1, "b1")), L.ptr(_f32c(w2, "w2")), L.ptr(_f32c(b2, "b2")),
                                  L.ptr(gate), L.stream_ptr()), "ldn_se_gate_slots")
    return gate


def conv_rows_gated_fits(cin, gate_rows):
    return cin % 8 == 0 and cin <= 2048 and (255 // int(gate_rows) + 2) * ((int(cin) + 31) // 32 * 32) * 4 <= 44 * 1024


def conv_rows_gated(a2d, w, scale, shift, out2d, gate, gate_rows, *, m_count=None, m_cap=None, relu=1, relu_if_neg=None, out_rows=None,
                    residual2d=None):
    L.require_device(a2d, w, out2d, gate)
    lib = L.load()
    cout, t, cin = w.shape
    if t != 1:
        raise L.LdnError("conv_rows_gated: 1x1 weights expected")
    if gate.shape[1] != cin or not gate.is_contiguous():
        raise L.LdnError("conv_rows_gated: gate must be a contiguous [images, cin] tensor")
    if m_cap is None:
        m_cap = a2d.shape[0]
    if (m_cap + gate_rows - 1) // gate_rows > gate.shape[0]:
        raise L.LdnError("conv_rows_gated: gate has fewer rows than the images m_cap spans")
    L.check(lib.ldn_conv_rows_gated(L.ptr(_f32rows(a2d, "a")), a2d.stride(0), L.ptr(_i32c(m_count, "m_count")), m_cap,
                                    L.ptr(split_rows_weight(w)), cin, cout, L.ptr(_f32c(scale, "scale")), L.ptr(_f32c(shift, "shift")), relu,
                                    L.ptr(_i32c(relu_if_neg, "relu_if_neg")), L.ptr(_i32c(out_rows, "out_rows")),
                                    L.ptr(_f32rows(residual2d, "residual")), residual2d.stride(0) if residual2d is not None else 0,
                                    L.ptr(_f32rows(out2d, "out")), out2d.stride(0), L.ptr(_f32c(gate, "gate")), int(gate_rows),
                                    L.stream_ptr(out2d)), "ldn_conv_rows_gated")
    return out2d


def grouped_conv3x3_image(a_nhwc, w, group_width, ch_idx, ch_cnt, scale, shift, out_nhwc, *, stride=1, relu=1):
    L.require_device(a_nhwc, w, out_nhwc, ch_idx)
    lib = L.load()
    B, Hi, Wi, lda = a_nhwc.shape
    _, Ho, Wo, ldo = out_nhwc.shape
    C = w.shape[0]
    L.check(lib.ldn_grouped_conv3x3_image(L.ptr(_f32c(a_nhwc, "a")), lda, B, Hi, Wi, stride, Ho, Wo, L.ptr(_f32c(w, "w")), C,
                                          group_width, L.ptr(_i32c(ch_idx, "ch_idx")), L.ptr(_i32c(ch_cnt, "ch_cnt")),
                                          L.ptr(_f32c(scale, "scale")), L.ptr(_f32c(shift, "shift")), relu,
                                          L.ptr(_f32c(out_nhwc, "out")), ldo, L.stream_ptr(out_nhwc)), "ldn_grouped_conv3x3_image")
    return out_nhwc


def se_packed(a2d, row_prefix, w1, b1, w2, b2, max_rows_per_image, ch_idx=None, ch_cnt=None):
    L.require_device(a2d, row_prefix)
    lib = L.load()
    B = row_prefix.numel() - 1
    S, C = w1.shape
    work = _work(lib.ldn_se_packed_workspace_bytes(B, C, max_rows_per_image), a2d.device)
    L.check(lib.ldn_se_packed(L.ptr(_f32c(a2d, "a")), a2d.stride(0), L.ptr(_i32c(row_prefix, "row_prefix")), B, C, S,
                              L.ptr(_f32c(w1, "w1")), L.ptr(_f32c(b1, "b1")), L.ptr(_f32c(w2, "w2")), L.ptr(_f32c(b2, "b2")),
                              L.ptr(_i32c(ch_idx, "ch_idx")), L.ptr(_i32c(ch_cnt, "ch_cnt")), max_rows_per_image, L.ptr(work),
                              L.stream_ptr()), "ldn_se_packed")
    return a2d


def _hi_lo(w):
    hi = w.to(torch.bfloat16)
    lo = (w - hi.float()).to(torch.bfloat16)
    return hi, lo


def pack_w2_pairs(conv2_weight, f32=False):
    W = conv2_weight.shape[0]
    w = conv2_weight.detach().float().permute(2, 3, 1, 0).reshape(9, W // 2, 2, W // 2, 2)
    w = w.permute(0, 1, 3, 4, 2).contiguous()
    if f32:
        return w
    hi, lo = _hi_lo(w)
    return torch.stack((hi, lo), dim=-2).contiguous()


def pack_w3_pairs(w3_scaled, f32=False):
    cout, W = w3_scaled.shape
    w = w3_scaled.detach().float().t().reshape(W // 2, 2, cout).permute(0, 2, 1).contiguous()
    if f32:
        return w
    hi, lo = _hi_lo(w)
    return torch.stack((hi, lo), dim=-2).contiguous()


def pack_w1_split(conv1_weight_2d, f32=False):
    W, cin = conv1_weight_2d.shape
    if f32:
        return conv1_weight_2d.detach().float().contiguous()
    w = conv1_weight_2d.detach().float().reshape(W, cin // 8, 8)
    hi, lo = _hi_lo(w)
    return torch.stack((hi, lo), dim=-2).contiguous()


def bottleneck_head(x_nhwc, w1_split, ch_idx, ch_cnt, scale1, shift1, post_sub1, h1_split, x_split=None):
    L.require_device(x_nhwc, w1_split, h1_split)
    lib = L.load()
    B, H, Wd, cin = x_nhwc.shape
    width = ch_idx.shape[1]
    if w1_split.dtype == torch.float32:
        if not w1_split.is_contiguous() or x_split is not None:
            raise L.LdnError("bottleneck_head: the fp32 form takes a contiguous fp32 weight matrix and writes no x_split")
        L.check(lib.ldn_bottleneck_head_f32(L.ptr(_f32c(x_nhwc, "x")), cin, B, H * Wd, cin, L.ptr(w1_split), width,
                                            L.ptr(_i32c(ch_idx, "ch_idx")), L.ptr(_i32c(ch_cnt, "ch_cnt")), L.ptr(_f32c(scale1, "scale1")),
                                            L.ptr(_f32c(shift1, "shift1")), L.ptr(_f32c(post_sub1, "post_sub1")),
                                            L.ptr(_f32c(h1_split, "h1")), h1_split.shape[-1], L.stream_ptr(h1_split)), "ldn_bottleneck_head_f32")
        return h1_split
    if w1_split.dtype != torch.bfloat16 or not w1_split.is_contiguous():
        raise L.LdnError("bottleneck_head: w1_split must be the contiguous bf16 tensor of pack_w1_split")
    if x_split is not None:
        if x_split.dtype != torch.float32 or not x_split.is_contiguous() or x_split.numel() * 4 < lib.ldn_x_split_bytes(B * H * Wd, cin):
            raise L.LdnError("bottleneck_head: x_split must be a contiguous fp32 buffer of x_split_buffer(B * H * W, cin)")
        L.check(lib.ldn_bottleneck_head_split(L.ptr(_f32c(x_nhwc, "x")), cin, B, H * Wd, cin, L.ptr(w1_split), width,
                                              L.ptr(_i32c(ch_idx, "ch_idx")), L.ptr(_i32c(ch_cnt, "ch_cnt")), L.ptr(_f32c(scale1, "scale1")),
                                              L.ptr(_f32c(shift1, "shift1")), L.ptr(_f32c(post_sub1, "post_sub1")),
                                              L.ptr(_f32c(h1_split, "h1")), h1_split.shape[-1], L.ptr(x_split),
                                              L.stream_ptr(h1_split)), "ldn_bottleneck_head_split")
        return h1_split
    L.check(lib.ldn_bottleneck_head(L.ptr(_f32c(x_nhwc, "x")), cin, B, H * Wd, cin, L.ptr(w1_split), width,
                                    L.ptr(_i32c(ch_idx, "ch_idx")), L.ptr(_i32c(ch_cnt, "ch_cnt")), L.ptr(_f32c(scale1, "scale1")),
                                    L.ptr(_f32c(shift1, "shift1")), L.ptr(_f32c(post_sub1, "post_sub1")),
                                    L.ptr(_f32c(h1_split, "h1")), h1_split.shape[-1], L.stream_ptr(h1_split)), "ldn_bottleneck_head")
    return h1_split


CHAIN_BLOCK_FIELDS = 14


def chain_table(rows, device):
    flat = []
    for row in rows:
        if len(row) != CHAIN_BLOCK_FIELDS:
            raise L.LdnError("chain_table: a block takes 14 tensors")
        for t in row:
            if t is not None and (not t.is_contiguous() or t.device != torch.device(device)):
                raise L.LdnError("chain_table: tensors must be contiguous and on the table's device")
            flat.append(0 if t is None else t.data_ptr())
    return torch.tensor(flat, dtype=torch.int64).view(len(rows), CHAIN_BLOCK_FIELDS).to(device)


def bottleneck_chain(x_in, x_work, table, width, hidden, G, gran, gap_in, f32=False):
    L.require_device(x_in, x_work, table, gap_in)
    lib = L.load()
    B, H, Wd, C = x_in.shape
    n = table.shape[0]
    dev = x_in.device
    if x_work.shape != x_in.shape or not (x_in.is_contiguous() and x_work.is_contiguous()) or x_in.dtype != torch.float32:
        raise L.LdnError("bottleneck_chain: x_in / x_work must be contiguous fp32 NHWC tensors of the same shape")
    if table.dtype != torch.int64 or table.dim() != 2 or table.shape[1] != CHAIN_BLOCK_FIELDS or not table.is_contiguous():
        raise L.LdnError("bottleneck_chain: table must come from chain_table")
    if gap_in.dim() != 3 or gap_in.shape[0] != B or gap_in.shape[2] != C:
        raise L.LdnError("bottleneck_chain: gap_in must be [B, splits, C]")
    masks = torch.empty(n, B, G, device=dev, dtype=torch.float32)
    ch_idx = torch.empty(n, B, width, device=dev, dtype=torch.int32)
    ch_cnt = torch.empty(n, B, device=dev, dtype=torch.int32)
    colsum = torch.empty(B, 8, C, device=dev, dtype=torch.float32)
    h1 = torch.empty(B, H, Wd, width, device=dev, dtype=torch.float32)
    L.check((lib.ldn_bottleneck_chain_f32 if f32 else lib.ldn_bottleneck_chain)(L.ptr(x_in), L.ptr(x_work), C, B, H, Wd, C, width, L.ptr(table), n, hidden, G, gran,
                                     L.ptr(_f32c(gap_in, "gap_in")), gap_in.shape[1], L.ptr(colsum), L.ptr(masks), L.ptr(ch_idx),
                                     L.ptr(ch_cnt), L.ptr(h1), width, L.stream_ptr(x_work)), "ldn_bottleneck_chain")
    return masks, ch_idx, ch_cnt, colsum


def bottleneck_chain_fits(H, W, C, width, hidden, G):
    return bool(L.load().ldn_bottleneck_chain_fits(H, W, C, width, hidden, G))


def bottleneck_tail_splits(H, W, width, stride=1):
    return L.load().ldn_bottleneck_tail_splits(H, W, width, stride)


def bottleneck_tail(h1_split, w2_pairs, w3_pairs, ch_idx, ch_cnt, scale2, shift2_tab, post_sub2, shift3, out_nhwc, *,
                    residual=None, colsum=None, stride=1):
    L.require_device(h1_split, w2_pairs, w3_pairs, out_nhwc)
    lib = L.load()
    B, H, Wd, ldh = h1_split.shape
    width = ch_idx.shape[1]
    cout = out_nhwc.shape[-1]
    Ho, Wo = (H - 1) // stride + 1, (Wd - 1) // stride + 1
    if tuple(out_nhwc.shape) != (B, Ho, Wo, cout) or (residual is not None and tuple(residual.shape[:3]) != (B, Ho, Wo)):
        raise L.LdnError(f"bottleneck_tail: out / residual must be [B={B}, {Ho}, {Wo}, cout] for an {H}x{Wd} input at stride {stride}")
    if w2_pairs.dtype != w3_pairs.dtype or w2_pairs.dtype not in (torch.bfloat16, torch.float32) or not (w2_pairs.is_contiguous() and w3_pairs.is_contiguous()):
        raise L.LdnError("bottleneck_tail: w2_pairs / w3_pairs must be the contiguous tensors of pack_w2_pairs / pack_w3_pairs (both bf16, or both fp32)")
    fn = lib.ldn_bottleneck_tail if w2_pairs.dtype == torch.bfloat16 else lib.ldn_bottleneck_tail_f32
    L.check(fn(L.ptr(_f32c(h1_split, "h1")), ldh, B, H, Wd, stride, width, L.ptr(w2_pairs), L.ptr(w3_pairs), cout,
                                    L.ptr(_i32c(ch_idx, "ch_idx")), L.ptr(_i32c(ch_cnt, "ch_cnt")), L.ptr(_f32c(scale2, "scale2")),
                                    L.ptr(_f32c(shift2_tab, "shift2_tab")), L.ptr(_f32c(post_sub2, "post_sub2")),
                                    L.ptr(_f32c(shift3, "shift3")), L.ptr(residual),
                                    residual.shape[-1] if residual is not None else 0, L.ptr(_f32c(out_nhwc, "out")), cout,
                                    L.ptr(colsum), L.stream_ptr(out_nhwc)), "ldn_bottleneck_tail")
    return out_nhwc


def x_split_buffer(pixels, cin, dev):
    return torch.empty(L.load().ldn_x_split_bytes(pixels, cin) // 4, device=dev, dtype=torch.float32)


def decode_x_split(xs, pixels, cin):
    t = xs.view(torch.bfloat16).reshape(-1, cin // 16, 2, 2, 32, 8).float()
    v = (t[:, :, :, 0] + t[:, :, :, 1]).permute(0, 3, 1, 2, 4).reshape(-1, cin)
    return v[:pixels]


def bottleneck_tail_proj_fits(H, W, width, cin):
    return bool(L.load().ldn_bottleneck_tail_proj_fits(H, W, width, cin))


def bottleneck_tail_proj(h1_split, w2_pairs, w3_pairs, ch_idx, ch_cnt, scale2, shift2_tab, post_sub2, shift3d, x_split, wd_pairs,
                         out_nhwc, *, colsum=None):
    L.require_device(h1_split, w2_pairs, w3_pairs, x_split, wd_pairs, out_nhwc)
    lib = L.load()
    B, H, Wd, ldh = h1_split.shape
    width = ch_idx.shape[1]
    cout = out_nhwc.shape[-1]
    cin = wd_pairs.shape[0] * 2
    if tuple(out_nhwc.shape) != (B, H, Wd, cout) or x_split.numel() * 4 < lib.ldn_x_split_bytes(B * H * Wd, cin) or not x_split.is_contiguous():
        raise L.LdnError(f"bottleneck_tail_proj: out must be [B={B}, {H}, {Wd}, cout], x_split the buffer bottleneck_head filled")
    for t in (w2_pairs, w3_pairs, wd_pairs):
        if t.dtype != torch.bfloat16 or not t.is_contiguous():
            raise L.LdnError("bottleneck_tail_proj: w2_pairs / w3_pairs / wd_pairs must be the contiguous bf16 tensors of pack_w2_pairs / pack_w3_pairs")
    L.check(lib.ldn_bottleneck_tail_proj(L.ptr(_f32c(h1_split, "h1")), ldh, B, H, Wd, width, L.ptr(w2_pairs), L.ptr(w3_pairs), cout,
                                         L.ptr(_i32c(ch_idx, "ch_idx")), L.ptr(_i32c(ch_cnt, "ch_cnt")), L.ptr(_f32c(scale2, "scale2")),
                                         L.ptr(_f32c(shift2_tab, "shift2_tab")), L.ptr(_f32c(post_sub2, "post_sub2")),
                                         L.ptr(_f32c(shift3d, "shift3d")), L.ptr(x_split), cin, L.ptr(wd_pairs),
                                         L.ptr(_f32c(out_nhwc, "out")), cout, L.ptr(colsum), L.stream_ptr(out_nhwc)), "ldn_bottleneck_tail_proj")
    return out_nhwc


def bottleneck_smallmap_fits(H, W, cin, width, cout):
    return bool(L.load().ldn_bottleneck_smallmap_fits(H, W, cin, width, cout))


def bottleneck_smallmap(x_nhwc, w1_split, w2_pairs, w3_pairs, ch_idx, ch_cnt, scale1, shift1, post_sub1, scale2, shift2_tab, post_sub2,
                        shift3, out_nhwc, *, residual=None, colsum=None):
    L.require_device(x_nhwc, w1_split, w2_pairs, w3_pairs, out_nhwc)
    lib = L.load()
    B, H, Wd, cin = x_nhwc.shape
    width = ch_idx.shape[1]
    cout = out_nhwc.shape[-1]
    if tuple(out_nhwc.shape) != (B, H, Wd, cout) or (residual is not None and tuple(residual.shape) != (B, H, Wd, cout)):
        raise L.LdnError(f"bottleneck_smallmap: out / residual must be [B={B}, {H}, {Wd}, cout]")
    if colsum is not None and (tuple(colsum.shape) != (B, 2, cout) or not colsum.is_contiguous()):
        raise L.LdnError("bottleneck_smallmap: colsum must be a contiguous [B, 2, cout] tensor")
    for w in (w1_split, w2_pairs, w3_pairs):
        if w.dtype != torch.bfloat16 or not w.is_contiguous():
            raise L.LdnError("bottleneck_smallmap: weights must be the contiguous bf16 tensors of pack_w1_split / pack_w2_pairs / pack_w3_pairs")
    L.check(lib.ldn_bottleneck_smallmap(L.ptr(_f32c(x_nhwc, "x")), cin, B, H, Wd, cin, width, L.ptr(w1_split), L.ptr(w2_pairs),
                                        L.ptr(w3_pairs), cout, L.ptr(_i32c(ch_idx, "ch_idx")), L.ptr(_i32c(ch_cnt, "ch_cnt")),
                                        L.ptr(_f32c(scale1, "scale1")), L.ptr(_f32c(shift1, "shift1")), L.ptr(_f32c(post_sub1, "post_sub1")),
                                        L.ptr(_f32c(scale2, "scale2")), L.ptr(_f32c(shift2_tab, "shift2_tab")),
                                        L.ptr(_f32c(post_sub2, "post_sub2")), L.ptr(_f32c(shift3, "shift3")), L.ptr(residual),
                                        cout if residual is not None else 0, L.ptr(_f32c(out_nhwc, "out")), cout, L.ptr(colsum),
                                        L.stream_ptr(out_nhwc)), "ldn_bottleneck_smallmap")
    return out_nhwc


def pack_stem_weights(w_scaled):
    cout = w_scaled.shape[0]
    if tuple(w_scaled.shape[1:]) != (3, 7, 7) or cout % 32:
        raise L.LdnError("pack_stem_weights: expected [cout % 32 == 0, 3, 7, 7]")
    w = w_scaled.detach().float().permute(0, 2, 3, 1).reshape(cout, 7, 21)
    k = torch.zeros(cout, 8, 24, device=w.device, dtype=torch.float32)
    k[:, :7, :21] = w
    k = k.reshape(cout, 24, 8)[:, :22]
    k = k.reshape(cout // 32, 32, 11, 2, 8)
    k = k.permute(0, 2, 3, 1, 4).reshape(cout // 32, 11, 64, 8)
    hi, lo = _hi_lo(k)
    return torch.stack((hi, lo), dim=-2).contiguous()


def stem_conv_pool(x_nhwc, w_frag, shift, cout, want_gap=False):
    L.require_device(x_nhwc, w_frag, shift)
    lib = L.load()
    B, H, W, cin = x_nhwc.shape
    if cin != 3 or x_nhwc.dtype != torch.float32 or not x_nhwc.is_contiguous():
        raise L.LdnError("stem_conv_pool: x must be a contiguous fp32 [B,H,W,3] tensor")
    if w_frag.dtype != torch.bfloat16 or not w_frag.is_contiguous() or w_frag.numel() * 2 != lib.ldn_stem_weight_bytes(cout):
        raise L.LdnError("stem_conv_pool: w_frag must be the contiguous bf16 tensor of pack_stem_weights")
    Hc, Wc = (H - 1) // 2 + 1, (W - 1) // 2 + 1
    Hp, Wp = (Hc - 1) // 2 + 1, (Wc - 1) // 2 + 1
    out = torch.empty(B, Hp, Wp, cout, device=x_nhwc.device, dtype=torch.float32)
    if want_gap:
        gap = torch.empty(B, lib.ldn_stem_gap_splits(H, W), cout, device=x_nhwc.device, dtype=torch.float32)
        L.check(lib.ldn_stem_conv_pool_gap(L.ptr(x_nhwc), B, H, W, L.ptr(w_frag), L.ptr(_f32c(shift, "shift")), cout, L.ptr(out), Hp, Wp,
                                           L.ptr(gap), L.stream_ptr(out)), "ldn_stem_conv_pool_gap")
        return out, gap
    L.check(lib.ldn_stem_conv_pool(L.ptr(x_nhwc), B, H, W, L.ptr(w_frag), L.ptr(_f32c(shift, "shift")), cout, L.ptr(out), Hp, Wp,
                                   L.stream_ptr(out)), "ldn_stem_conv_pool")
    return out


def pack_stem3_weights(w_scaled):
    cout = w_scaled.shape[0]
    if tuple(w_scaled.shape[1:]) != (3, 3, 3) or cout % 32:
        raise L.LdnError("pack_stem3_weights: expected [cout % 32 == 0, 3, 3, 3]")
    k = torch.zeros(cout, 3, 16, device=w_scaled.device, dtype=torch.float32)
    k[:, :, :9] = w_scaled.detach().float().permute(0, 2, 3, 1).reshape(cout, 3, 9)
    k = k.reshape(cout // 32, 32, 3, 2, 8).permute(0, 2, 3, 1, 4).reshape(cout // 32, 3, 64, 8)
    hi, lo = _hi_lo(k)
    return torch.stack((hi, lo), dim=-2).contiguous()


def stem3_conv(x_nhwc, w_frag, shift, cout, relu=True):
    L.require_device(x_nhwc, w_frag, shift)
    lib = L.load()
    B, H, W, cin = x_nhwc.shape
    if cin != 3 or x_nhwc.dtype != torch.float32 or not x_nhwc.is_contiguous():
        raise L.LdnError("stem3_conv: x must be a contiguous fp32 [B,H,W,3] tensor")
    if w_frag.dtype != torch.bfloat16 or not w_frag.is_contiguous() or w_frag.numel() * 2 != lib.ldn_stem3_weight_bytes(cout):
        raise L.LdnError("stem3_conv: w_frag must be the contiguous bf16 tensor of pack_stem3_weights")
    Ho, Wo = (H - 1) // 2 + 1, (W - 1) // 2 + 1
    out = torch.empty(B, Ho, Wo, cout, device=x_nhwc.device, dtype=torch.float32)
    L.check(lib.ldn_stem3_conv(L.ptr(x_nhwc), B, H, W, L.ptr(w_frag), L.ptr(_f32c(shift, "shift")), cout, int(bool(relu)),
                               L.ptr(out), Ho, Wo, L.stream_ptr(out)), "ldn_stem3_conv")
    return out


def token_lists(keep):
    B, Lt = keep.shape
    ix = mask_to_index(keep.reshape(B, Lt, 1).float().contiguous(), Lt, 1, 1)
    return ix.idx3, ix.pre3, ix.cnt[0:1]


def packed_mha(qkv2d, tok_rows, prefix, B, heads, max_tokens, scale=None, head_keep=None):
    L.require_device(qkv2d, tok_rows, prefix)
    lib = L.load()
    rows, three_dim = qkv2d.shape
    dim = three_dim // 3
    d = dim // heads
    if three_dim != 3 * dim or dim != heads * d or qkv2d.dtype != torch.float32 or qkv2d.stride(1) != 1:
        raise L.LdnError("packed_mha: qkv must be fp32 [rows, 3 * heads * head_dim]")
    out = torch.empty(rows, dim, device=qkv2d.device, dtype=torch.float32)
    if head_keep is not None:
        if tuple(head_keep.shape) != (B, heads):
            raise L.LdnError("packed_mha: head_keep must be [B, heads]")
        L.check(lib.ldn_packed_mha_heads(L.ptr(qkv2d), qkv2d.stride(0), L.ptr(_i32c(tok_rows, "tok_rows")), L.ptr(_i32c(prefix, "prefix")), B,
                                         heads, d, max_tokens, float(scale if scale is not None else d ** -0.5),
                                         L.ptr(_f32c(head_keep, "head_keep")), L.ptr(out), dim, L.stream_ptr(out)), "ldn_packed_mha_heads")
        return out
    L.check(lib.ldn_packed_mha(L.ptr(qkv2d), qkv2d.stride(0), L.ptr(_i32c(tok_rows, "tok_rows")), L.ptr(_i32c(prefix, "prefix")), B, heads,
                               d, max_tokens, float(scale if scale is not None else d ** -0.5), L.ptr(out), dim, L.stream_ptr(out)),
            "ldn_packed_mha")
    return out
```

Before: 22880.

## Fuse successor block's conv1 into bottleneck tail epilogue and add dense h1 input

```diff
diff --git a/include/ldn_hip.h b/include/ldn_hip.h
--- a/include/ldn_hip.h
+++ b/include/ldn_hip.h
@@ -141,6 +141,12 @@
                              const void* w3_pairs, int cout, const int32_t* ch_idx, const int32_t* ch_cnt, const float* scale2,
                              const float* shift2_tab, const float* post_sub2, const float* shift3d, const void* x_split,
                              int cin, const void* wd_pairs, float* out, int ldo, float* colsum, void* stream);
+int ldn_bottleneck_tail_next(const void* h1, int ldh, int h1_dense, int B, int H, int Wd, int stride, int width, const void* w2_pairs,
+                             const void* w3_pairs, int cout, const int32_t* ch_idx, const int32_t* ch_cnt, const float* scale2,
+                             const float* shift2_tab, const float* post_sub2, const float* shift3, const float* residual, int ldr,
+                             const void* x_split, int cin, const void* wd_pairs, float* out, int ldo, float* colsum,
+                             const void* w1_next, int wn, const float* scale1n, const float* shift1n, const float* post_sub1n,
+                             void* h1_next, int ldhn, void* stream);
 
 int ldn_bottleneck_smallmap_fits(int H, int Wd, int cin, int width, int cout);
 int ldn_bottleneck_smallmap(const float* x, int ldx, int B, int H, int Wd, int cin, int width, const void* w1_split,
diff --git a/laudnet_amd/_lib.py b/laudnet_amd/_lib.py
--- a/laudnet_amd/_lib.py
+++ b/laudnet_amd/_lib.py
@@ -77,6 +77,7 @@
     "ldn_bottleneck_head_split": ([_P, _I, _I, _I, _I, _P, _I, _P, _P, _P, _P, _P, _P, _I, _P, _P], _I),
     "ldn_bottleneck_tail_proj_fits": ([_I, _I, _I, _I], _I),
     "ldn_bottleneck_tail_proj": ([_P, _I, _I, _I, _I, _I, _P, _P, _I, _P, _P, _P, _P, _P, _P, _P, _I, _P, _P, _I, _P, _P], _I),
+    "ldn_bottleneck_tail_next": ([_P, _I, _I, _I, _I, _I, _I, _I, _P, _P, _I, _P, _P, _P, _P, _P, _P, _P, _I, _P, _I, _P, _P, _I, _P, _P, _I, _P, _P, _P, _P, _I, _P], _I),
     "ldn_stem_weight_bytes": ([_I], C.c_size_t),
     "ldn_stem_conv_pool": ([_P, _I, _I, _I, _P, _P, _I, _P, _I, _I, _P], _I),
     "ldn_stem_gap_splits": ([_I, _I], _I),
diff --git a/laudnet_amd/csrc/ldn_tail.hip b/laudnet_amd/csrc/ldn_tail.hip
--- a/laudnet_amd/csrc/ldn_tail.hip
+++ b/laudnet_amd/csrc/ldn_tail.hip
@@ -22,6 +22,8 @@
     int rows_per_blk, mblocks;
     int slice_bytes;
     const unsigned char* pxs; const unsigned char* pw;
+    const unsigned char* w1n; const float* sc1n; const float* sh1n; const float* ps1n;
+    unsigned char* h1n; long h1n_row_bytes;
 };
 constexpr int T_PROJ_CIN = 64;
 
@@ -137,15 +139,16 @@
             } \
 }
 
-template <int NS, int ST = 1, bool PROJ = false, bool F32 = false>
+template <int NS, int ST = 1, bool PROJ = false, bool F32 = false, int NH = 0, bool DENSE = false>
 __device__ __forceinline__ void tail_body(const TailArgs& p, const int b, const int mb, unsigned char* const smem, const int tid) {
     static_assert(!PROJ || (NS == 2 && ST == 1), "the folded projection exists for the 64-wide stride-1 block (stage 1's first block)");
     static_assert(!(PROJ && F32), "the folded projection is a bf16x3 form");
+    static_assert(!((NH > 0 || DENSE) && (F32 || NS == 8)) && !(DENSE && (ST == 2 || PROJ)), "next-head / dense-h1 forms: bf16x3, widths 64 and 128, dense h1 at stride 1");
     constexpr int W = NS * 32;
     constexpr int SLICE_BUFS = ST == 2 ? 2 : (NS == 2 ? 1 : 2);
     constexpr int W2_ROW = NS * 256;
     constexpr int W2_SLOT = 16 * W2_ROW;
-    constexpr int CW = (NS == 8 || PROJ) ? 32 : 64;
+    constexpr int CW = (NS == 8 || PROJ || NH > 0) ? 32 : 64;
     constexpr int NCS = CW / 32;
     constexpr int W3_ROW = CW * 8;
     constexpr int RPI = 1024 / W3_ROW;
@@ -158,6 +161,11 @@
     unsigned char* const s_w3 = smem + T_KIDX_BYTES;
     float* const s_tab = reinterpret_cast<float*>(s_w3 + 2 * W3_SLOT);
     unsigned char* const s_scr = reinterpret_cast<unsigned char*>(s_tab + 18 * NP);
+    constexpr int WN = NH * 32;
+    constexpr int W1T = 128 * WN;
+    constexpr int W1B = PROJ ? 1 : 2;
+    unsigned char* const s_w1n = s_scr + 8 * 4096;
+    float* const s_sh3 = reinterpret_cast<float*>(s_w1n + W1B * W1T);
 
     int lane = tid & 63;
     const int wave = __builtin_amdgcn_readfirstlane(tid >> 6);
@@ -222,6 +230,21 @@
 
     const unsigned lds_h1 = lds_off(s_h1), lds_w2 = lds_off(s_w2), lds_w3 = lds_off(s_w3);
     auto dma_h1 = [&](int slice, int q) {
+        if constexpr (DENSE) {
+#pragma unroll
+            for (int i = 0; i < 4; ++i) {
+                const int q2 = 4 * q + i;
+                int ln = lane;
+                asm volatile("" : "+v"(ln));
+                const int r = 2 * q2 + (ln >> 5), d = ln & 31;
+                const int lsl = (d >> 2) ^ (q2 & 7);
+                const int ch = s_kidx[2 * (slice * 16 + (lsl >> 1) * 4 + (d & 3))];
+                const unsigned char* src = (r < NR && ch >= 0) ? p.h1 + (in_row0 + r) * p.h1_row_bytes + (ch >> 1) * 8 + (lsl & 1) * 4
+                                                               : reinterpret_cast<const unsigned char*>(g_tail_zero);
+                dma4_touch(src, lds_h1 + (slice % SLICE_BUFS) * p.slice_bytes + q2 * 256);
+            }
+            return;
+        }
         const int r = q * 8 + (lane >> 3);
         const int lslot = (lane & 7) ^ ((r >> 1) & 7);
         const unsigned char* src = r < NR ? p.h1 + (in_row0 + r) * p.h1_row_bytes + slice * 128 + lslot * 16
@@ -454,7 +477,20 @@
             }
         }
     };
-    if (nchunk3 > 0) dma_w3(0);
+    const unsigned lds_w1n = lds_off(s_w1n);
+    auto dma_w1n = [&](int cc) {
+        if constexpr (NH > 0)
+            for (int i = wave; i < W1T / 1024; i += 8) dma16(p.w1n + (long)cc * W1T + i * 1024 + lane * 16, lds_w1n + (cc % W1B) * W1T + i * 1024);
+    };
+    if (nchunk3 > 0) { dma_w3(0); if (W1B == 2) dma_w1n(0); }
+    f32x16 h1acc[NH > 0 ? NH : 1];
+    if constexpr (NH > 0) {
+#pragma unroll
+        for (int j = 0; j < NH; ++j)
+#pragma unroll
+            for (int r = 0; r < 16; ++r) h1acc[j][r] = 0.f;
+        for (int i = tid; i < p.cout; i += 512) s_sh3[i] = p.sh3[i];
+    }
 
     for (int i = tid; i < NP; i += 512) {
         const int ch = i < Kb ? s_kidx[i] : -1;
@@ -536,7 +572,8 @@
     }
     for (int cc = 0; cc < nchunk3; ++cc) {
         if (cc == 0) { wait_vm<0>(); lds_barrier(); }
-        if (cc + 1 < nchunk3) dma_w3(cc + 1);
+        if (cc + 1 < nchunk3) { dma_w3(cc + 1); if (W1B == 2) dma_w1n(cc + 1); }
+        if (W1B == 1) dma_w1n(cc);
         const unsigned char* ws = s_w3 + (cc & 1) * W3_SLOT;
 #pragma unroll
         for (int cs = 0; cs < NCS; ++cs) {
@@ -545,12 +582,18 @@
             if constexpr (!PROJ) {
 #pragma unroll
             for (int it = 0; it < 4; ++it) {
+                if constexpr (NH > 0) {
+                    const int prow = wave * 32 + l31;
+                    const float* src = (p.residual && prow < npix) ? p.residual + (size_t)(out_row0 + prow) * p.ldr + c0 + 8 * it + 4 * h : g_tail_zero;
+                    res[it] = *reinterpret_cast<const f32x4*>(src);
+                } else {
                 const int prow = wave * 32 + trw + 8 * it;
                 const float* src = (p.residual && prow < npix) ? p.residual + (size_t)(out_row0 + prow) * p.ldr + c0 + tc * 4 : g_tail_zero;
                 res[it] = __builtin_nontemporal_load(reinterpret_cast<const f32x4*>(src));
-            }
-            }
-            f32x4 sh = *reinterpret_cast<const f32x4*>(p.sh3 + c0 + tc * 4);
+                }
+            }
+            }
+            f32x4 sh = *reinterpret_cast<const f32x4*>(NH > 0 ? g_tail_zero : p.sh3 + c0 + tc * 4);
             f32x16 acc3;
             TT(ta)
 #pragma unroll
@@ -603,7 +646,19 @@
             TT(tb)
             TT_ADD(w3k, ta, tb)
             if (cs == NCS - 1) wait_vm<0>();
-            if constexpr (PROJ) asm volatile("" : "+v"(sh));
+            if constexpr (NH > 0) {
+                if (W1B == 1) lds_barrier();
+#pragma unroll
+                for (int q4 = 0; q4 < 4; ++q4) {
+                    const f32x4 s4 = *reinterpret_cast<const f32x4*>(s_sh3 + c0 + 8 * q4 + 4 * h);
+#pragma unroll
+                    for (int e = 0; e < 4; ++e) {
+                        float x = acc3[4 * q4 + e] + s4[e];
+                        if constexpr (!PROJ) x = x + res[PROJ ? 0 : q4][e];
+                        acc3[4 * q4 + e] = fmaxf(x, 0.f);
+                    }
+                }
+            } else if constexpr (PROJ) asm volatile("" : "+v"(sh));
             else asm volatile("" : "+v"(res[0]), "+v"(res[PROJ ? 0 : 1]), "+v"(res[PROJ ? 0 : 2]), "+v"(res[PROJ ? 0 : 3]), "+v"(sh));
             TT(ta)
             TT_ADD(w3wait, tb, ta)
@@ -619,10 +674,12 @@
             for (int it = 0; it < 4; ++it) {
                 const int row = trw + 8 * it, prow = wave * 32 + row;
                 f32x4 x = *reinterpret_cast<const f32x4*>(scr + row * 32 + ((tc ^ (row & 7)) << 2));
+                if constexpr (NH == 0) {
                 if constexpr (PROJ) x = x + sh;
                 else x = x + sh + res[PROJ ? 0 : it];
 #pragma unroll
                 for (int e = 0; e < 4; ++e) x[e] = fmaxf(x[e], 0.f);
+                }
                 if (prow < npix) {
                     __builtin_nontemporal_store(x, reinterpret_cast<f32x4*>(p.out + (size_t)(out_row0 + prow) * p.ldo + c0 + tc * 4));
                     csum += x;
@@ -636,6 +693,31 @@
             }
             asm volatile("s_waitcnt lgkmcnt(0)" ::: "memory");
             __builtin_amdgcn_wave_barrier();
+            if constexpr (NH > 0) {
+                if (active) {
+                    bf16x8 nbh[2], nbl[2];
+#pragma unroll
+                    for (int t = 0; t < 2; ++t)
+#pragma unroll
+                        for (int i = 0; i < 8; ++i) {
+                            const float x = acc3[8 * t + i];
+                            const __bf16 hb = (__bf16)x;
+                            nbh[t][i] = hb;
+                            nbl[t][i] = (__bf16)(x - (float)hb);
+                        }
+                    const unsigned char* wt = s_w1n + (cc % W1B) * W1T + (unsigned)(2 * h * WN + l31) * 16;
+#pragma unroll
+                    for (int jn = 0; jn < NH; ++jn)
+#pragma unroll
+                        for (int t = 0; t < 2; ++t) {
+                            const bf16x8 ah = *reinterpret_cast<const bf16x8*>(wt + ((4 * t) * WN + 32 * jn) * 16);
+                            const bf16x8 al = *reinterpret_cast<const bf16x8*>(wt + ((4 * t + 1) * WN + 32 * jn) * 16);
+                            h1acc[jn] = t_mfma_bf16(al, nbh[t], h1acc[jn]);
+                            h1acc[jn] = t_mfma_bf16(ah, nbl[t], h1acc[jn]);
+                            h1acc[jn] = t_mfma_bf16(ah, nbh[t], h1acc[jn]);
+                        }
+                }
+            }
             TT(tb)
             TT_ADD(w3epi, ta, tb)
         }
@@ -643,6 +725,32 @@
         lds_barrier();
         TT(tb)
         TT_ADD(w3bar, ta, tb)
+    }
+    if constexpr (NH > 0) {
+        const int pmn = wave * 32 + l31;
+        if (active && pmn < npix) {
+            unsigned char* orow = p.h1n + (out_row0 + pmn) * p.h1n_row_bytes;
+#pragma unroll
+            for (int jn = 0; jn < NH; ++jn)
+#pragma unroll
+                for (int q4 = 0; q4 < 4; ++q4) {
+                    const int n0 = 32 * jn + 8 * q4 + 4 * h;
+                    const f32x4 sc = *reinterpret_cast<const f32x4*>(p.sc1n + n0);
+                    const f32x4 sh = *reinterpret_cast<const f32x4*>(p.sh1n + n0);
+                    const f32x4 ps = *reinterpret_cast<const f32x4*>(p.ps1n + n0);
+                    u32x4 outv;
+#pragma unroll
+                    for (int d = 0; d < 2; ++d) {
+                        const float v0 = fmaxf(h1acc[jn][4 * q4 + 2 * d] * sc[2 * d] + sh[2 * d], 0.f) - ps[2 * d];
+                        const float v1 = fmaxf(h1acc[jn][4 * q4 + 2 * d + 1] * sc[2 * d + 1] + sh[2 * d + 1], 0.f) - ps[2 * d + 1];
+                        const bf16x2 hh = {(__bf16)v0, (__bf16)v1};
+                        const bf16x2 ll = {(__bf16)(v0 - (float)hh[0]), (__bf16)(v1 - (float)hh[1])};
+                        outv[2 * d] = __builtin_bit_cast(unsigned, hh);
+                        outv[2 * d + 1] = __builtin_bit_cast(unsigned, ll);
+                    }
+                    *reinterpret_cast<u32x4*>(orow + n0 * 4) = outv;
+                }
+        }
     }
 #ifdef LDN_TRACE
     TT(tr4)
@@ -654,10 +762,10 @@
 #endif
 }
 
-template <int NS, int ST, bool PROJ = false, bool F32 = false>
+template <int NS, int ST, bool PROJ = false, bool F32 = false, int NH = 0, bool DENSE = false>
 __global__ __launch_bounds__(512, ((NS == 2 && ST == 1) ? 4 : 2)) void k_tail(const TailArgs p) {
     extern __shared__ __attribute__((aligned(16))) unsigned char smem[];
-    tail_body<NS, ST, PROJ, F32>(p, blockIdx.x % p.B, blockIdx.x / p.B, smem, threadIdx.x);
+    tail_body<NS, ST, PROJ, F32, NH, DENSE>(p, blockIdx.x % p.B, blockIdx.x / p.B, smem, threadIdx.x);
 }
 
 LDN_DEFINE_TU_VIOLATIONS(tu_violations_tail)
@@ -695,19 +803,20 @@
     return best;
 }
 
-template <int NS, int ST, bool PROJ = false, bool F32 = false>
+template <int NS, int ST, bool PROJ = false, bool F32 = false, int NH = 0, bool DENSE = false>
 static int launch_tail(TailArgs& a, hipStream_t st) {
     constexpr int W = NS * 32;
     const int R = a.rows_per_blk;
     const int nr = tail_region_pixels(R, a.Hi, a.Wi, ST);
     a.slice_bytes = round_up((round_up(nr, 8) + 1) * 128, 1024);
     const size_t lds2 = tail_lds2(R, a.Hi, a.Wi, NS, ST);
-    const size_t lds3 = (size_t)T_KIDX_BYTES + 2 * (size_t)(W / 2 + (PROJ ? T_PROJ_CIN / 2 : 0)) * ((NS == 8 || PROJ) ? 32 : 64) * 8 + (size_t)18 * W * 4 + 8 * 4096;
+    const size_t lds3 = (size_t)T_KIDX_BYTES + 2 * (size_t)(W / 2 + (PROJ ? T_PROJ_CIN / 2 : 0)) * ((NS == 8 || PROJ || NH > 0) ? 32 : 64) * 8 + (size_t)18 * W * 4 + 8 * 4096
+                        + (NH > 0 ? (size_t)(PROJ ? 1 : 2) * 128 * 32 * NH + (size_t)a.cout * 4 : 0);
     const size_t lds = lds2 > lds3 ? lds2 : lds3;
     LDN_REQUIRE(lds <= 160 * 1024, "ldn_bottleneck_tail: %zu B of LDS exceed 160 KiB (map %dx%d, width %d)", lds, a.Ho, a.Wo, W);
     LDN_REQUIRE(ST == 2 || NS == 2 || round_up(nr, 8) / 8 <= 72, "ldn_bottleneck_tail: input region of %d pixels too large for the slice pipeline", nr);
-    LDN_REQUIRE(allow_dynamic_lds(reinterpret_cast<const void*>(&k_tail<NS, ST, PROJ, F32>), lds), "k_tail: cannot reserve %zu B of LDS", lds);
-    hipLaunchKernelGGL((k_tail<NS, ST, PROJ, F32>), dim3((unsigned)a.B * a.mblocks), dim3(512), lds, st, a);
+    LDN_REQUIRE(allow_dynamic_lds(reinterpret_cast<const void*>(&k_tail<NS, ST, PROJ, F32, NH, DENSE>), lds), "k_tail: cannot reserve %zu B of LDS", lds);
+    hipLaunchKernelGGL((k_tail<NS, ST, PROJ, F32, NH, DENSE>), dim3((unsigned)a.B * a.mblocks), dim3(512), lds, st, a);
     LDN_CHECK_LAUNCH("k_tail");
     return LDN_OK;
 }
@@ -743,7 +852,9 @@
                                 const void* w3_pairs, int cout, const int32_t* ch_idx, const int32_t* ch_cnt,
                                 const float* scale2, const float* shift2_tab, const float* post_sub2,
                                 const float* shift3, const float* residual, int ldr, float* out, int ldo,
-                                float* colsum, const void* x_split, const void* wd_pairs, bool f32, void* stream);
+                                float* colsum, const void* x_split, const void* wd_pairs, bool f32, void* stream,
+                                int h1_dense = 0, const void* w1n = nullptr, int wn = 0, const float* sc1n = nullptr, const float* sh1n = nullptr,
+                                const float* ps1n = nullptr, void* h1n = nullptr, int ldhn = 0);
 
 extern "C" int ldn_bottleneck_tail(const void* h1_split, int ldh, int B, int H, int Wd, int stride, int width, const void* w2_pairs,
                                    const void* w3_pairs, int cout, const int32_t* ch_idx, const int32_t* ch_cnt,
@@ -781,11 +892,26 @@
                                 post_sub2, shift3d, nullptr, 0, out, ldo, colsum, x_split, wd_pairs, false, stream);
 }
 
+extern "C" int ldn_bottleneck_tail_next(const void* h1, int ldh, int h1_dense, int B, int H, int Wd, int stride, int width, const void* w2_pairs,
+                                        const void* w3_pairs, int cout, const int32_t* ch_idx, const int32_t* ch_cnt,
+                                        const float* scale2, const float* shift2_tab, const float* post_sub2, const float* shift3,
+                                        const float* residual, int ldr, const void* x_split, int cin, const void* wd_pairs, float* out, int ldo,
+                                        float* colsum, const void* w1_next, int wn, const float* scale1n, const float* shift1n,
+                                        const float* post_sub1n, void* h1_next, int ldhn, void* stream) {
+    LDN_REQUIRE(h1_dense || w1_next, "ldn_bottleneck_tail_next: neither a dense h1 nor a successor (use ldn_bottleneck_tail)");
+    LDN_REQUIRE(!x_split == !wd_pairs && (!x_split || (!residual && width == 64 && cin == ldn::T_PROJ_CIN && stride == 1 && (uintptr_t)x_split % 16 == 0 && (uintptr_t)wd_pairs % 16 == 0)),
+                "ldn_bottleneck_tail_next: the folded projection takes x_split and wd_pairs, no residual, width 64, cin 64, stride 1");
+    return bottleneck_tail_impl(h1, ldh, B, H, Wd, stride, width, w2_pairs, w3_pairs, cout, ch_idx, ch_cnt, scale2, shift2_tab, post_sub2, shift3,
+                                residual, ldr, out, ldo, colsum, x_split, wd_pairs, false, stream, h1_dense ? 1 : 0, w1_next, wn, scale1n, shift1n,
+                                post_sub1n, h1_next, ldhn);
+}
+
 static int bottleneck_tail_impl(const void* h1_split, int ldh, int B, int H, int Wd, int stride, int width, const void* w2_pairs,
                                 const void* w3_pairs, int cout, const int32_t* ch_idx, const int32_t* ch_cnt,
                                 const float* scale2, const float* shift2_tab, const float* post_sub2,
                                 const float* shift3, const float* residual, int ldr, float* out, int ldo,
-                                float* colsum, const void* x_split, const void* wd_pairs, bool f32, void* stream) {
+                                float* colsum, const void* x_split, const void* wd_pairs, bool f32, void* stream,
+                                int h1_dense, const void* w1n, int wn, const float* sc1n, const float* sh1n, const float* ps1n, void* h1n, int ldhn) {
     LDN_REQUIRE(h1_split && w2_pairs && w3_pairs && ch_idx && ch_cnt && scale2 && shift2_tab && post_sub2 && shift3 && out,
                 "ldn_bottleneck_tail: null pointer");
     LDN_REQUIRE(width == 64 || width == 128 || width == 256, "ldn_bottleneck_tail: width must be 64, 128 or 256 (got %d)", width);
@@ -811,6 +937,31 @@
     a.rows_per_blk = tail_rows_per_block(H, Wd, width / 32, stride, &a.mblocks);
     LDN_REQUIRE(a.rows_per_blk > 0, "ldn_bottleneck_tail: a %dx%d map of width %d (stride %d) does not fit the workgroup (ldn_bottleneck_tail_splits == 0)", H, Wd, width, stride);
     hipStream_t st = static_cast<hipStream_t>(stream);
+    if (h1_dense || w1n) {
+        LDN_REQUIRE(!f32 && (width == 64 || width == 128), "ldn_bottleneck_tail_next: bf16x3 arithmetic, width 64 or 128 (got %d)", width);
+        LDN_REQUIRE(!h1_dense || (stride == 1 && !x_split), "ldn_bottleneck_tail_next: a dense h1 is read at stride 1, without the folded projection");
+        LDN_REQUIRE(cout % 32 == 0 && cout <= 2048, "ldn_bottleneck_tail_next: cout must be a multiple of 32, at most 2048");
+        if (w1n) {
+            LDN_REQUIRE(sc1n && sh1n && ps1n && h1n, "ldn_bottleneck_tail_next: null pointer");
+            LDN_REQUIRE((wn == 64 || wn == 128) && wn >= width && (width == 64 || wn == 128) && (stride == 1 || (width == 128 && !h1_dense)),
+                        "ldn_bottleneck_tail_next: successor width %d after a width-%d tail of stride %d is not built", wn, width, stride);
+            LDN_REQUIRE(ldhn >= wn && ldhn % 4 == 0, "ldn_bottleneck_tail_next: ldhn must be a multiple of 4 and >= wn");
+            LDN_REQUIRE((uintptr_t)w1n % 16 == 0 && (uintptr_t)sc1n % 16 == 0 && (uintptr_t)sh1n % 16 == 0 && (uintptr_t)ps1n % 16 == 0 && (uintptr_t)h1n % 16 == 0,
+                        "ldn_bottleneck_tail_next: pointers must be 16-byte aligned");
+            a.w1n = static_cast<const unsigned char*>(w1n); a.sc1n = sc1n; a.sh1n = sh1n; a.ps1n = ps1n;
+            a.h1n = static_cast<unsigned char*>(h1n); a.h1n_row_bytes = (long)ldhn * 4;
+        }
+        const int nh = w1n ? wn / 32 : 0;
+        if (width == 64) {
+            if (x_split) return nh == 2 ? launch_tail<2, 1, true, false, 2>(a, st) : launch_tail<2, 1, true, false, 4>(a, st);
+            if (h1_dense) return nh == 0 ? launch_tail<2, 1, false, false, 0, true>(a, st)
+                               : (nh == 2 ? launch_tail<2, 1, false, false, 2, true>(a, st) : launch_tail<2, 1, false, false, 4, true>(a, st));
+            return nh == 2 ? launch_tail<2, 1, false, false, 2>(a, st) : launch_tail<2, 1, false, false, 4>(a, st);
+        }
+        if (stride == 2) return launch_tail<4, 2, false, false, 4>(a, st);
+        if (h1_dense) return nh == 0 ? launch_tail<4, 1, false, false, 0, true>(a, st) : launch_tail<4, 1, false, false, 4, true>(a, st);
+        return launch_tail<4, 1, false, false, 4>(a, st);
+    }
     if (f32) {
         LDN_REQUIRE(!x_split, "ldn_bottleneck_tail: the folded projection is a bf16x3 form");
         if (stride == 2) {
diff --git a/laudnet_amd/ops.py b/laudnet_amd/ops.py
--- a/laudnet_amd/ops.py
+++ b/laudnet_amd/ops.py
@@ -844,6 +844,42 @@
     return torch.stack((hi, lo), dim=-2).contiguous()
 
 
+def pack_w1_next(conv1_weight_2d):
+    wn, cin = conv1_weight_2d.shape
+    if cin % 32 or wn % 32:
+        raise L.LdnError("pack_w1_next: wn and cin must be multiples of 32")
+    r = torch.arange(16).view(2, 1, 8)
+    c = ((r & 3) + 8 * (r >> 2) + 4 * torch.arange(2).view(1, 2, 1)).reshape(-1).to(conv1_weight_2d.device)
+    w = conv1_weight_2d.detach().float().reshape(wn, cin // 32, 32)[:, :, c].reshape(wn, cin // 32, 2, 2, 8)
+    w = w.permute(1, 2, 3, 0, 4).contiguous()
+    hi, lo = _hi_lo(w)
+    return torch.stack((hi, lo), dim=3).contiguous()
+
+
+def decode_h1_dense(h1_dense):
+    t = h1_dense.contiguous().view(torch.bfloat16).reshape(*h1_dense.shape[:-1], h1_dense.shape[-1] // 2, 2, 2).float()
+    return (t[..., 0, :] + t[..., 1, :]).reshape(h1_dense.shape)
+
+
+def _next_head_args(next_w1, next_scale1, next_shift1, next_post_sub1, next_h1, B, Ho, Wo, cout, what):
+    given = [t is not None for t in (next_w1, next_scale1, next_shift1, next_post_sub1, next_h1)]
+    if not any(given):
+        return None, 0, None, None, None, None, 0
+    if not all(given):
+        raise L.LdnError(f"{what}: next_w1, next_scale1, next_shift1, next_post_sub1 and next_h1 go together")
+    L.require_device(next_w1, next_h1)
+    if next_w1.dtype != torch.bfloat16 or not next_w1.is_contiguous() or next_w1.dim() != 6 or next_w1.shape[0] * 32 != cout:
+        raise L.LdnError(f"{what}: next_w1 must be the contiguous bf16 tensor of pack_w1_next for cin = cout = {cout}")
+    wn = next_w1.shape[4]
+    if tuple(next_h1.shape[:3]) != (B, Ho, Wo) or next_h1.shape[-1] < wn or next_h1.dtype != torch.float32 or not next_h1.is_contiguous():
+        raise L.LdnError(f"{what}: next_h1 must be a contiguous fp32 [B={B}, {Ho}, {Wo}, >= {wn}] buffer")
+    for t in (next_scale1, next_shift1, next_post_sub1):
+        if t.numel() != wn:
+            raise L.LdnError(f"{what}: next_scale1 / next_shift1 / next_post_sub1 must have {wn} entries")
+    return (L.ptr(next_w1), wn, L.ptr(_f32c(next_scale1, "next_scale1")), L.ptr(_f32c(next_shift1, "next_shift1")),
+            L.ptr(_f32c(next_post_sub1, "next_post_sub1")), L.ptr(next_h1), next_h1.shape[-1])
+
+
 def bottleneck_head(x_nhwc, w1_split, ch_idx, ch_cnt, scale1, shift1, post_sub1, h1_split, x_split=None):
     L.require_device(x_nhwc, w1_split, h1_split)
     lib = L.load()
@@ -922,7 +958,8 @@
 
 
 def bottleneck_tail(h1_split, w2_pairs, w3_pairs, ch_idx, ch_cnt, scale2, shift2_tab, post_sub2, shift3, out_nhwc, *,
-                    residual=None, colsum=None, stride=1):
+                    residual=None, colsum=None, stride=1, next_w1=None, next_scale1=None, next_shift1=None, next_post_sub1=None,
+                    next_h1=None, h1_dense=False):
     L.require_device(h1_split, w2_pairs, w3_pairs, out_nhwc)
     lib = L.load()
     B, H, Wd, ldh = h1_split.shape
@@ -933,6 +970,18 @@
         raise L.LdnError(f"bottleneck_tail: out / residual must be [B={B}, {Ho}, {Wo}, cout] for an {H}x{Wd} input at stride {stride}")
     if w2_pairs.dtype != w3_pairs.dtype or w2_pairs.dtype not in (torch.bfloat16, torch.float32) or not (w2_pairs.is_contiguous() and w3_pairs.is_contiguous()):
         raise L.LdnError("bottleneck_tail: w2_pairs / w3_pairs must be the contiguous tensors of pack_w2_pairs / pack_w3_pairs (both bf16, or both fp32)")
+    nxt = _next_head_args(next_w1, next_scale1, next_shift1, next_post_sub1, next_h1, B, Ho, Wo, cout, "bottleneck_tail")
+    if h1_dense or nxt[0] is not None:
+        if w2_pairs.dtype != torch.bfloat16:
+            raise L.LdnError("bottleneck_tail: the successor's conv1 / a dense h1 exist in bf16x3 arithmetic only")
+        L.check(lib.ldn_bottleneck_tail_next(L.ptr(_f32c(h1_split, "h1")), ldh, int(bool(h1_dense)), B, H, Wd, stride, width, L.ptr(w2_pairs),
+                                             L.ptr(w3_pairs), cout, L.ptr(_i32c(ch_idx, "ch_idx")), L.ptr(_i32c(ch_cnt, "ch_cnt")),
+                                             L.ptr(_f32c(scale2, "scale2")), L.ptr(_f32c(shift2_tab, "shift2_tab")),
+                                             L.ptr(_f32c(post_sub2, "post_sub2")), L.ptr(_f32c(shift3, "shift3")), L.ptr(residual),
+                                             residual.shape[-1] if residual is not None else 0, None, 0, None,
+                                             L.ptr(_f32c(out_nhwc, "out")), cout, L.ptr(colsum), *nxt, L.stream_ptr(out_nhwc)),
+                "ldn_bottleneck_tail_next")
+        return out_nhwc
     fn = lib.ldn_bottleneck_tail if w2_pairs.dtype == torch.bfloat16 else lib.ldn_bottleneck_tail_f32
     L.check(fn(L.ptr(_f32c(h1_split, "h1")), ldh, B, H, Wd, stride, width, L.ptr(w2_pairs), L.ptr(w3_pairs), cout,
                                     L.ptr(_i32c(ch_idx, "ch_idx")), L.ptr(_i32c(ch_cnt, "ch_cnt")), L.ptr(_f32c(scale2, "scale2")),
@@ -958,7 +1007,7 @@
 
 
 def bottleneck_tail_proj(h1_split, w2_pairs, w3_pairs, ch_idx, ch_cnt, scale2, shift2_tab, post_sub2, shift3d, x_split, wd_pairs,
-                         out_nhwc, *, colsum=None):
+                         out_nhwc, *, colsum=None, next_w1=None, next_scale1=None, next_shift1=None, next_post_sub1=None, next_h1=None):
     L.require_device(h1_split, w2_pairs, w3_pairs, x_split, wd_pairs, out_nhwc)
     lib = L.load()
     B, H, Wd, ldh = h1_split.shape
@@ -970,6 +1019,15 @@
     for t in (w2_pairs, w3_pairs, wd_pairs):
         if t.dtype != torch.bfloat16 or not t.is_contiguous():
             raise L.LdnError("bottleneck_tail_proj: w2_pairs / w3_pairs / wd_pairs must be the contiguous bf16 tensors of pack_w2_pairs / pack_w3_pairs")
+    nxt = _next_head_args(next_w1, next_scale1, next_shift1, next_post_sub1, next_h1, B, H, Wd, cout, "bottleneck_tail_proj")
+    if nxt[0] is not None:
+        L.check(lib.ldn_bottleneck_tail_next(L.ptr(_f32c(h1_split, "h1")), ldh, 0, B, H, Wd, 1, width, L.ptr(w2_pairs), L.ptr(w3_pairs), cout,
+                                             L.ptr(_i32c(ch_idx, "ch_idx")), L.ptr(_i32c(ch_cnt, "ch_cnt")), L.ptr(_f32c(scale2, "scale2")),
+                                             L.ptr(_f32c(shift2_tab, "shift2_tab")), L.ptr(_f32c(post_sub2, "post_sub2")),
+                                             L.ptr(_f32c(shift3d, "shift3d")), None, 0, L.ptr(x_split), cin, L.ptr(wd_pairs),
+                                             L.ptr(_f32c(out_nhwc, "out")), cout, L.ptr(colsum), *nxt, L.stream_ptr(out_nhwc)),
+                "ldn_bottleneck_tail_next")
+        return out_nhwc
     L.check(lib.ldn_bottleneck_tail_proj(L.ptr(_f32c(h1_split, "h1")), ldh, B, H, Wd, width, L.ptr(w2_pairs), L.ptr(w3_pairs), cout,
                                          L.ptr(_i32c(ch_idx, "ch_idx")), L.ptr(_i32c(ch_cnt, "ch_cnt")), L.ptr(_f32c(scale2, "scale2")),
                                          L.ptr(_f32c(shift2_tab, "shift2_tab")), L.ptr(_f32c(post_sub2, "post_sub2")),
```

New measurement: 22600. 1.2% lower.
